# deepseek-ai/DeepEP

Measured on AMD Instinct MI355X. Metric: combine GB/s (device-resident BF16 top-k weighted reduce) at 1/2/4/8 MI355X, higher is better.
Workload: dtype bf16; 1 GPU; EP=1 combine, 8192 tokens/rank x hidden 7168 x top-8, 256 experts, uniform routing, expanded layout, gating-weighted; hidden=7168, topk=8, experts=256, accumulate=fp32, parallelism=ep1

## Files before the change

deepep_amd/_lib.py:

```python
import ctypes
import hashlib
import os
import threading
from typing import Optional

_HERE = os.path.dirname(os.path.abspath(__file__))
LIB_PATH = os.environ.get('DEEPEP_AMD_LIB', os.path.join(_HERE, 'libdeepep_amd.so'))
SOURCES = [os.path.join(_HERE, 'csrc', f) for f in ('combine.hip', 'dispatch.hip', 'symmetric.hip', 'plan.hip',
                                                      'fp8_cast.hip', 'fault.h')]
HEADER = os.path.join(os.path.dirname(_HERE), 'include', 'deepep_amd.h')
HIPCC_FLAGS = ['--offload-arch=gfx950', '-O3', '-fPIC', '-std=c++17', '-Wall']


def source_build_id() -> Optional[str]:
    if not all(os.path.exists(p) for p in SOURCES + [HEADER]):
        return None
    h = hashlib.sha256(' '.join(HIPCC_FLAGS).encode())
    for p in SOURCES + [HEADER]:
        h.update(os.path.basename(p).encode())
        with open(p, 'rb') as f:
            h.update(f.read())
    return h.hexdigest()[:16]


def binary_build_id(path: str) -> Optional[str]:
    if not os.path.exists(path):
        return None
    with open(path, 'rb') as f:
        data = f.read()
    i = data.find(b'DEEPEP_BUILD_ID=')
    return data[i + 16:i + 32].decode(errors='replace') if i >= 0 else None
ABI_VERSION = 14

MODE_LOCAL, MODE_EPILOGUE, MODE_FUSED = 0, 1, 2

ERROR_RECORD_INTS = 8
FLAG_BAD_SLOT, FLAG_TIMEOUT, FLAG_BAD_ADDRESS = 1, 2, 4
FAULT_NAMES = {1: 'scatter row outside every window', 2: 'plan window row past its window',
               3: 'plan unit / received row out of range', 4: 'dispatch row past its destination buffer'}


def describe_error_record(rec) -> str:
    rec = [int(v) for v in rec]
    bits = [n for b, n in ((FLAG_BAD_SLOT, 'rejected slot / unit'), (FLAG_TIMEOUT, 'barrier timeout'),
                           (FLAG_BAD_ADDRESS, 'address outside every window')) if rec[0] & b]
    text = f'error flag {rec[0]} ({", ".join(bits) or "none"})'
    if len(rec) > 6 and rec[1]:
        addr = (rec[5] & 0xffffffff) << 32 | (rec[4] & 0xffffffff)
        text += (f'; first fault: {FAULT_NAMES.get(rec[1], rec[1])}, unit/row {rec[2]}, rank/lane {rec[3]}, '
                 f'address {addr:#x}, extent {rec[6]}')
    return text

PLAN_BLOCK_TOKENS = 64
DISPATCH_BLOCK_ROWS = 128
PLAN_EXPANDED, PLAN_SINGLE, PLAN_INTERLEAVE, PLAN_RANK_LAYOUT, PLAN_WINDOW, PLAN_LOCAL_BYPASS = 1, 2, 4, 8, 16, 32

_lib = None
_lock = threading.Lock()

_P = ctypes.c_void_p
_I = ctypes.c_int
_I64 = ctypes.c_int64

SIGNATURES = {
    'deepep_amd_abi_version': (_I, []),
    'deepep_amd_last_error': (ctypes.c_char_p, []),
    'deepep_amd_build_id': (ctypes.c_char_p, []),
    'deepep_combine_reduce': (_I, [_I, _I,
                                   _P, _I64, _I64,
                                   _P, _I64, _I,
                                   _P,
                                   _P, _P,
                                   _P, _I64,
                                   _I, _I,
                                   _P, _I64,
                                   _P, _P, _I,
                                   _I64, _I,
                                   _I, _P,
                                   _P]),
    'deepep_build_local_plan': (_I, [_P, _I, _I, _I, _I, _P, _I, _I, _P, _P, _P]),
    'deepep_set_launch_config': (_I, [_I, _I]),
    'deepep_combine_buffer_size': (_I64, [_I, _I, _I, _I, _I]),
    'deepep_dispatch_route': (_I, [_P, _I, _I, _I, _I, _P, _P, _P, _P]),
    'deepep_dispatch_notify': (_I, [_P, _I, _I, _I, _I, _I, _P, _P, _P, _P, _I64, _P]),
    'deepep_dispatch_notify_workspace': (_I64, [_I, _I, _I]),
    'deepep_dispatch_receive': (_I, [_P, _I64, _I, _I, _I, _I, _I, _I, _P, _I, _I, _P, _I, _I, _P, _P, _P, _P, _I, _I, _P,
                                     _P, _P, _P]),
    'deepep_dispatch_expert_counts': (_I, [_P, _I, _I, _I, _P, _P]),
    'deepep_dispatch_pack': (_I, [_P, _I64, _I, _P, _I64, _I, _P, _P, _I, _I, _I, _P, _P, _I,
                                  _P, _P, _I64, _I64, _I, _I, _I, _I, _P, _P]),
    'deepep_cast_fp8': (_I, [_P, _I64, _I, _I, _I, _P, _P, _P]),
    'deepep_dispatch_pack_cast': (_I, [_P, _I64, _I, _I, _P, _P, _I, _I, _I, _P, _P, _I,
                                       _P, _P, _I64, _I64, _I, _I, _I, _I, _P, _P]),
    'deepep_dispatch_count': (_I, [_P, _I64, _I, _I, _I, _I, _I, _I, _P, _I, _I, _P, _I, _I, _P, _P, _P, _P, _P]),
    'deepep_dispatch_scan': (_I, [_P, _I, _I, _I, _I, _P, _P, _P]),
    'deepep_dispatch_slots': (_I, [_P, _I64, _I, _I, _I, _I, _I, _P, _P, _P, _P, _P]),
    'deepep_dispatch_copy': (_I, [_P, _I64, _I, _I, _I, _I, _I, _I, _P, _I, _P, _I64, _P, _I64, _I,
                                  _P, _P, _P, _I64, _P, _P, _P, _I, _P, _P, _P]),
    'deepep_route_block_counts': (_I, [_P, _I, _I, _I, _I, _I, _P, _P, _P]),
    'deepep_plan_expert': (_I, [_P, _I, _I, _I, _I, _I, _P, _P, _I, _I, _I, _P, _P, _P, _I64, _I64, _P, _P, _I,
                                _P]),
    'deepep_plan_source': (_I, [_P, _I, _I, _I, _I, _I, _I, _P, _P, _P, _I, _I, _I, _I64, _I64, _P, _I, _P, _I, _P]),
    'deepep_sym_alloc': (_I, [_I64, ctypes.POINTER(ctypes.c_void_p)]),
    'deepep_sym_free': (_I, [_P]),
    'deepep_sym_export': (_I, [_P, _P]),
    'deepep_sym_import': (_I, [_P, ctypes.POINTER(ctypes.c_void_p)]),
    'deepep_sym_close': (_I, [_P]),
    'deepep_sym_barrier': (_I, [_P, _I, _I, _I64, _I64, _P, _P]),
    'deepep_sym_put': (_I, [_P, _I64, _P, _I, _I64, _I64, _P, _P]),
    'deepep_sym_signal': (_I, [_P, _I, _I, _I, _I64, _P]),
    'deepep_sym_wait': (_I, [_P, _I, _I, _I, _I64, _I64, _P, _P]),
    'deepep_stream_create_cu_budget': (_I, [_I, ctypes.POINTER(ctypes.c_void_p)]),
    'deepep_stream_destroy': (_I, [_P]),
    'deepep_stream_probe_cus': (_I, [_P, ctypes.POINTER(ctypes.c_int), ctypes.POINTER(ctypes.c_int)]),
    'deepep_combine_reduce_scatter': (_I, [_I, _P, _I64, _I64, _P, _I64, _I, _P, _P, _I, _I, _P, _I64, _P, _I,
                                           _I64, _I, _P, _I, _I64, _P, _P]),
}


class LibraryMissing(RuntimeError):
    pass


def load(path: Optional[str] = None):
    global _lib
    with _lock:
        if _lib is not None and path is None:
            return _lib
        p = path or LIB_PATH
        if not os.path.exists(p):
            raise LibraryMissing(f'deepep_amd: HIP library not found at {p}; run __graft_entry__.build()')
        want = source_build_id() if path is None and 'DEEPEP_AMD_LIB' not in os.environ else None
        if want is not None and binary_build_id(p) != want:
            raise RuntimeError(f'deepep_amd: {p} was built from other sources (build id {binary_build_id(p)}, '
                               f'sources {want}); run __graft_entry__.build()')
        lib = ctypes.CDLL(p)
        for name, (res, args) in SIGNATURES.items():
            fn = getattr(lib, name)
            fn.restype = res
            fn.argtypes = args
        version = lib.deepep_amd_abi_version()
        if version != ABI_VERSION:
            raise RuntimeError(f'deepep_amd: ABI version {version} != expected {ABI_VERSION}')
        if path is None:
            _lib = lib
        return lib


def check(rc: int, what: str) -> None:
    if rc != 0:
        msg = load().deepep_amd_last_error().decode(errors='replace')
        raise RuntimeError(f'deepep_amd: {what} failed ({rc}): {msg}')


def ptr(t) -> Optional[int]:
    return None if t is None else t.data_ptr()
```

deepep_amd/buffer.py:

```python
import math
import os
from typing import List, Optional, Sequence, Tuple, Union

import torch
import torch.distributed as dist

from .event import EventHandle, EventOverlap
from .exchange import ExchangeMixin
from .handle import BlockCounts, CombinePlan, EPHandle, build_ep_plan, chunk_geometry
from ._lib import DISPATCH_BLOCK_ROWS
from .kernels import MODE_EPILOGUE, MODE_FUSED, MODE_LOCAL, RowLayout
from .utils import align, ceil_div, check_torch_deterministic, value_or

topk_idx_t = torch.int32 if int(os.environ.get('EP_NUM_TOPK_IDX_BITS', 64)) == 32 else torch.int64

BUFFER_ALIGNMENT = 2 * 1024 * 1024
_BUDGET_STREAMS = {}
_TOKEN_ALIGN = 32


def _assert(cond: bool, msg: str = '') -> None:
    if not cond:
        raise RuntimeError(f'Assertion failed: {msg}')


def _token_bytes(hidden_bytes: int, sf_bytes: int, num_topk: int, with_metadata: bool) -> int:
    meta = num_topk * 8 + ((1 + num_topk) * 4 if with_metadata else 0)
    return (align(hidden_bytes, _TOKEN_ALIGN) + align(sf_bytes, _TOKEN_ALIGN) + align(meta, _TOKEN_ALIGN))


def calculate_buffer_size(num_ranks: int, num_max_tokens_per_rank: int, hidden: int, num_topk: int,
                          use_fp8_dispatch: bool, allow_multiple_reduction: bool) -> int:
    _assert(num_max_tokens_per_rank > 0 and hidden > 0, 'num_max_tokens_per_rank > 0 and hidden > 0')
    num_topk = 32 if num_topk == 0 else num_topk
    elem = 1 if use_fp8_dispatch else 2
    num_sf_packs = ceil_div(hidden, 32) if use_fp8_dispatch else 0
    dispatch_bytes = num_ranks * num_max_tokens_per_rank * _token_bytes(hidden * elem, num_sf_packs * 4, num_topk, True)
    slots = min(num_ranks, num_topk) if allow_multiple_reduction else num_topk
    combine_bytes = slots * num_max_tokens_per_rank * _token_bytes(hidden * 2, 0, num_topk, False)
    return align(max(dispatch_bytes, combine_bytes), BUFFER_ALIGNMENT)


def notify_layout(notify: List[int], num_ranks: int, rank: int, experts_per_rank: int, all_gathered: bool,
                  num_blocks: int = 0):
    R, r, w = num_ranks, rank, 1 + experts_per_rank + 2 * num_blocks
    if all_gathered:
        grid = [[notify[(s * R + d) * w:(s * R + d + 1) * w] for d in range(R)] for s in range(R)]
        rows = [grid[s][r] for s in range(R)]
        sends = [grid[r][d][0] for d in range(R)]
        offsets = [sum(grid[s][d][0] for s in range(r)) for d in range(R)]
    else:
        rows = [notify[i * w:(i + 1) * w] for i in range(R)]
        sends, offsets = None, None
    recv = [row[0] for row in rows]
    experts = [sum(row[1 + e] for row in rows) for e in range(experts_per_rank)]
    blocks = [list(row[1 + experts_per_rank:]) for row in rows]
    return sends, recv, experts, offsets, blocks


class ElasticBuffer(ExchangeMixin):

    def __init__(self,
                 group: dist.ProcessGroup,
                 num_bytes: Optional[int] = None,
                 num_cpu_bytes: int = 0,
                 num_max_tokens_per_rank: int = 0,
                 hidden: int = 0,
                 num_topk: int = 0,
                 use_fp8_dispatch: bool = False,
                 deterministic: bool = False,
                 allow_hybrid_mode: bool = True,
                 allow_multiple_reduction: bool = True,
                 prefer_overlap_with_compute: bool = True,
                 sl_idx: int = 3,
                 num_allocated_qps: int = 0,
                 num_cpu_timeout_secs: int = 300, num_gpu_timeout_secs: int = 100,
                 explicitly_destroy: bool = False):
        self.group = group
        self.rank_idx = group.rank()
        self.num_ranks = group.size()
        self.allow_hybrid_mode = allow_hybrid_mode
        self.allow_multiple_reduction = allow_multiple_reduction
        self.prefer_overlap_with_compute = prefer_overlap_with_compute
        self.deterministic = deterministic
        _assert(num_cpu_bytes == 0, 'CPU buffer segments (Engram storage) are not supported by this build')
        if num_bytes is None:
            num_bytes = calculate_buffer_size(self.num_ranks, num_max_tokens_per_rank, hidden, num_topk,
                                              use_fp8_dispatch, allow_multiple_reduction)
        _assert(num_bytes % BUFFER_ALIGNMENT == 0, 'num_bytes must be aligned to 2 MB')
        if os.environ.get('EP_BUFFER_DEBUG', 0):
            print(f'Initializing EP elastic buffer with {num_bytes} bytes at rank EP {self.rank_idx}/{self.num_ranks}')
        self.num_bytes = num_bytes
        self.num_max_tokens_per_rank = num_max_tokens_per_rank
        if num_allocated_qps == 0:
            num_allocated_qps = 17 if not allow_hybrid_mode else 65
        self.num_allocated_qps = num_allocated_qps
        self.num_cpu_timeout_secs = num_cpu_timeout_secs
        self.num_gpu_timeout_secs = num_gpu_timeout_secs
        self.explicitly_destroy = explicitly_destroy
        self.num_scaleout_ranks, self.num_scaleup_ranks = 1, self.num_ranks
        self.scaleout_rank_idx, self.scaleup_rank_idx = 0, self.rank_idx
        self.num_rdma_ranks, self.num_nvlink_ranks = 1, self.num_ranks
        self.use_cuda = torch.cuda.is_available()
        self.device = torch.device('cuda', torch.cuda.current_device()) if self.use_cuda else torch.device('cpu')
        self.comm_stream = torch.cuda.Stream(device=self.device) if self.use_cuda else None
        self._kernels = None
        self.runtime = self
        self._phase_events = None
        self._phase_unpipelined = False
        self.transport = os.environ.get('DEEPEP_TRANSPORT', 'rccl')
        _assert(self.transport in ('rccl', 'xgmi'), 'DEEPEP_TRANSPORT must be rccl or xgmi')
        self.local_bypass = os.environ.get('DEEPEP_LOCAL_BYPASS', '1') != '0'
        self.phase_a_cus = int(os.environ.get('DEEPEP_PHASE_A_CUS', 0))
        self.combine_cu_mode = os.environ.get('DEEPEP_COMBINE_CUS', 'chip')
        _assert(self.combine_cu_mode in ('chip', 'handle'), 'DEEPEP_COMBINE_CUS must be chip or handle')
        self._sym = None
        self._sym_gen = None
        self._old_sym_gens = set()
        self._capturing = False
        self._sym_exchange = None
        self._group_barrier()
        if self.transport == 'xgmi' and self.num_ranks > 1 and self.use_cuda and \
                int(os.environ.get('DEEPEP_EAGER_WINDOW', 1)) and not hasattr(group, 'comm'):
            self._window(self._window_bytes(hidden, num_topk, num_max_tokens_per_rank), slots=1, rows_per_slot=1)

    class _HostCopy:

        def __init__(self, src: torch.Tensor, pinned: torch.Tensor, stream):
            self.buf = pinned[:src.numel()]
            self.buf.copy_(src, non_blocking=True)
            self.event = torch.cuda.Event()
            self.event.record(stream)

        def wait(self) -> List[int]:
            self.event.synchronize()
            return self.buf.tolist()

    def _host_copy(self, src: torch.Tensor, stream) -> '_HostCopy':
        n = src.numel()
        prev = getattr(self, '_host_copy_last', None)
        if prev is not None:
            prev.event.synchronize()
        if getattr(self, '_pinned', None) is None or self._pinned.numel() < n:
            self._pinned = torch.empty((max(n, 4096),), dtype=torch.int32, pin_memory=True)
        self._host_copy_last = ElasticBuffer._HostCopy(src, self._pinned, stream)
        return self._host_copy_last

    def _group_barrier(self) -> None:
        if self.use_cuda:
            torch.cuda.synchronize()
        if isinstance(self.group, dist.ProcessGroup):
            dist.barrier(group=self.group)
        else:
            self.group.barrier()
        if self.use_cuda:
            torch.cuda.synchronize()

    def _window_bytes(self, hidden: int, num_topk: int, num_max_tokens: int) -> int:
        if hidden <= 0 or num_max_tokens <= 0:
            return 0
        from .handle import packed_row_layout
        K = num_topk or 32
        R = self.num_ranks
        slots, single = (min(R, K), False) if self.allow_multiple_reduction else (K, True)
        combine = slots * num_max_tokens * packed_row_layout(hidden, K, True, single)[0]
        dispatch = R * num_max_tokens * max(RowLayout.make(hidden * 2, 0, K).row_bytes,
                                            RowLayout.make(hidden, ceil_div(hidden, 128) * 4, K).row_bytes)
        return max(combine, dispatch)

    @property
    def kernels(self):
        if self._kernels is None:
            from .kernels import HipKernels
            self._kernels = HipKernels()
        return self._kernels

    def destroy(self) -> None:
        assert self.explicitly_destroy
        if self.runtime is not None:
            if self.use_cuda:
                torch.cuda.synchronize()
            if self._sym is not None:
                self._group_barrier()
                self._sym.destroy()
                self._sym = None
            self.runtime = None

    @staticmethod
    def get_buffer_size_hint(group: dist.ProcessGroup, num_max_tokens_per_rank: int, hidden: int,
                             num_topk: int = 0, use_fp8_dispatch: bool = False,
                             allow_hybrid_mode: bool = True, allow_multiple_reduction: bool = True) -> int:
        return calculate_buffer_size(group.size(), num_max_tokens_per_rank, hidden, num_topk,
                                     use_fp8_dispatch, allow_multiple_reduction)

    @staticmethod
    def get_elastic_buffer_alignment() -> int:
        return BUFFER_ALIGNMENT

    def barrier(self, use_comm_stream: bool = True, with_cpu_sync: bool = False, sequential: bool = True) -> None:
        self._note_capture()
        if with_cpu_sync and self.use_cuda:
            torch.cuda.synchronize()
        rccl = isinstance(self.group, dist.ProcessGroup) and dist.get_backend(self.group) == 'nccl'
        if self.use_cuda and (self._sym is not None or rccl):
            compute = torch.cuda.current_stream()
            stream = self.comm_stream if use_comm_stream else compute
            if stream != compute:
                stream.wait_stream(compute)
            if self._sym is not None:
                if not self._capturing:
                    self._sym.poll()
                self._sym.barrier(stream)
                if not self._capturing:
                    self._sym.publish(stream)
            else:
                with torch.cuda.stream(stream):
                    dist.all_reduce(torch.zeros(1, dtype=torch.int32, device=self.device), group=self.group)
            if stream != compute:
                compute.wait_stream(stream)
        elif isinstance(self.group, dist.ProcessGroup):
            dist.barrier(group=self.group)
        else:
            self.group.barrier()
        if with_cpu_sync and self.use_cuda:
            torch.cuda.synchronize()

    @staticmethod
    def capture() -> EventHandle:
        return EventHandle()

    def get_comm_stream(self) -> torch.cuda.Stream:
        return self.comm_stream

    def get_physical_domain_size(self) -> Tuple[int, int]:
        return self.num_rdma_ranks, self.num_nvlink_ranks

    def get_logical_domain_size(self) -> Tuple[int, int]:
        return self.num_scaleout_ranks, self.num_scaleup_ranks

    def get_theoretical_num_sms(self, num_experts: int, num_topk: int, num_scaleout_topk: int = 0,
                                rdma_gbs: float = 0, nvlink_gbs: float = 0,
                                sm_read_gbs: float = 200, sm_write_gbs: float = 50) -> int:
        assert num_scaleout_topk == 0
        key = (num_experts, num_topk, rdma_gbs, nvlink_gbs, sm_read_gbs, sm_write_gbs, self.prefer_overlap_with_compute,
               os.environ.get('EP_XGMI_GBS'))
        memo = self.__dict__.setdefault('_num_sms_memo', {})
        if key in memo:
            return memo[key]
        nvlink_gbs = nvlink_gbs or float(os.environ.get('EP_XGMI_GBS', 7 * 64))
        num_device_sms = torch.cuda.get_device_properties(self.device).multi_processor_count if self.use_cuda else 256

        def expected_topk(groups: int) -> float:
            return groups * (1 - math.comb(num_experts - num_experts // groups, num_topk) / math.comb(num_experts, num_topk))

        num_sms = num_device_sms
        if self.num_ranks > 1:
            e_topk = expected_topk(self.num_ranks)
            sm_read = 1 / e_topk
            sm_write = self.num_nvlink_ranks / self.num_ranks
            traffic = self.num_nvlink_ranks / self.num_ranks * (1 - 1 / self.num_nvlink_ranks)
            num_sms = max(nvlink_gbs / traffic * sm_read / sm_read_gbs, nvlink_gbs / traffic * sm_write / sm_write_gbs)
        num_sms = align(max(4, math.ceil(num_sms * 1.25)), 2)
        num_sms = num_sms if self.prefer_overlap_with_compute else max(num_sms, 64)
        memo[key] = min(num_sms, num_device_sms)
        return memo[key]

    def get_theoretical_num_qps(self, num_sms: int) -> int:
        num_qps = min(num_sms, 8 + 1)
        if self.allow_hybrid_mode:
            num_qps = num_sms * 16 + 1
        return min(num_qps, self.num_allocated_qps)

    def _sync_mode(self, previous_event, previous_event_before_epilogue, async_with_compute_stream,
                   allocate_on_comm_stream) -> bool:
        return (not async_with_compute_stream and previous_event is None and
                previous_event_before_epilogue is None and not allocate_on_comm_stream)

    def _note_capture(self) -> None:
        self._capturing = self.use_cuda and torch.cuda.is_current_stream_capturing()

    def _prologue(self, previous_event: Optional[EventHandle], allocate_on_comm_stream: bool):
        if not self.use_cuda:
            return None
        compute_stream = torch.cuda.current_stream()
        if allocate_on_comm_stream:
            torch.cuda.set_stream(self.comm_stream)
        if previous_event is not None:
            _assert(allocate_on_comm_stream, 'previous_event requires allocate_on_comm_stream')
            previous_event.stream_wait(self.comm_stream)
        else:
            self.comm_stream.wait_stream(compute_stream)
        return compute_stream

    def _before_epilogue(self, previous_event_before_epilogue: Optional[EventHandle]) -> None:
        if previous_event_before_epilogue is not None and self.use_cuda:
            previous_event_before_epilogue.stream_wait(self.comm_stream)

    def _epilogue(self, tensors: Sequence[Optional[torch.Tensor]], compute_stream,
                  allocate_on_comm_stream: bool, async_with_compute_stream: bool) -> Optional[EventHandle]:
        if not self.use_cuda:
            return None
        event = None
        if async_with_compute_stream:
            event = EventHandle(self.comm_stream)
            if int(os.environ.get('EP_AVOID_RECORD_STREAM', 0)):
                event.tensors_to_record = list(tensors)
            else:
                for t in tensors:
                    if t is not None and t.is_cuda:
                        t.record_stream(compute_stream)
                        t.record_stream(self.comm_stream)
        else:
            compute_stream.wait_stream(self.comm_stream)
        if allocate_on_comm_stream:
            torch.cuda.set_stream(compute_stream)
        return event

    def _mark(self, stream) -> None:
        if self._phase_events is not None and self.use_cuda:
            ev = torch.cuda.Event(enable_timing=True)
            ev.record(stream)
            self._phase_events.append(ev)

    @staticmethod
    def _null_ctx():
        import contextlib
        return contextlib.nullcontext()

    def _stream_ctx(self):
        if self.use_cuda:
            return torch.cuda.stream(self.comm_stream)
        import contextlib
        return contextlib.nullcontext()

    def _a2a(self, out: torch.Tensor, inp: torch.Tensor, out_splits: Optional[List[int]] = None,
             in_splits: Optional[List[int]] = None) -> None:
        if self.num_ranks == 1:
            out.copy_(inp)
            return
        dist.all_to_all_single(out, inp, out_splits, in_splits, group=self.group)

    def _all_to_all(self, out: torch.Tensor, inp: torch.Tensor, out_splits: List[int], in_splits: List[int]) -> None:
        o = out.view(torch.uint8).view(out.shape[0], out.shape[1] * out.element_size())
        i = inp.view(torch.uint8).view(inp.shape[0], inp.shape[1] * inp.element_size())
        self._a2a(o, i, out_splits, in_splits)

    def dispatch(self,
                 x: Union[torch.Tensor, Tuple[torch.Tensor, torch.Tensor]],
                 topk_idx: Optional[torch.Tensor] = None,
                 topk_weights: Optional[torch.Tensor] = None,
                 cumulative_local_expert_recv_stats: Optional[torch.Tensor] = None,
                 num_experts: Optional[int] = None,
                 num_max_tokens_per_rank: Optional[int] = None,
                 expert_alignment: Optional[int] = None,
                 num_sms: int = 0, num_qps: int = 0,
                 previous_event: Optional[EventHandle] = None,
                 previous_event_before_epilogue: Optional[EventHandle] = None,
                 async_with_compute_stream: bool = False,
                 allocate_on_comm_stream: bool = False,
                 handle: Optional[EPHandle] = None,
                 do_handle_copy: bool = True,
                 do_cpu_sync: Optional[bool] = None,
                 do_expand: bool = False,
                 do_zero_padding: bool = False,
                 use_tma_aligned_col_major_sf: bool = False):
        check_torch_deterministic()
        args = (x, topk_idx, topk_weights, cumulative_local_expert_recv_stats, num_experts, num_max_tokens_per_rank,
                expert_alignment, num_sms, num_qps, previous_event, previous_event_before_epilogue,
                async_with_compute_stream, allocate_on_comm_stream, handle, do_handle_copy, do_cpu_sync, do_expand,
                do_zero_padding, use_tma_aligned_col_major_sf)
        budget = self._cu_budget_stream(num_sms)
        if budget is not None and self.use_cuda and torch.cuda.current_stream() == budget:
            budget = None
        if budget is None:
            return self._dispatch(*args)
        capturing = torch.cuda.is_current_stream_capturing()
        saved, self.comm_stream = self.comm_stream, budget
        if not capturing:
            budget.wait_stream(saved)
        try:
            return self._dispatch(*args, force_comm_stream=True)
        finally:
            self.comm_stream = saved
            if not capturing:
                saved.wait_stream(budget)

    def _dispatch(self, x, topk_idx, topk_weights, cumulative_local_expert_recv_stats, num_experts,
                  num_max_tokens_per_rank, expert_alignment, num_sms, num_qps, previous_event,
                  previous_event_before_epilogue, async_with_compute_stream, allocate_on_comm_stream, handle,
                  do_handle_copy, do_cpu_sync, do_expand, do_zero_padding, use_tma_aligned_col_major_sf,
                  force_comm_stream: bool = False):
        num_topk = (handle.topk_idx if topk_idx is None else topk_idx).shape[1]
        num_sms = self.get_theoretical_num_sms(num_experts or handle.num_experts, num_topk) if num_sms == 0 else num_sms
        num_qps = self.get_theoretical_num_qps(num_sms) if num_qps == 0 else num_qps
        _assert(num_qps <= self.num_allocated_qps, 'Allocated QPs are not enough')
        x, sf = x if isinstance(x, tuple) else (x, None)
        if handle is not None:
            _assert(topk_idx is None, 'topk_idx must be None with a cached handle')
            _assert(do_cpu_sync is None or not do_cpu_sync, 'Cannot do CPU sync with cached handle')
            topk_idx = handle.topk_idx
            num_max_tokens_per_rank = value_or(num_max_tokens_per_rank, handle.num_max_tokens_per_rank)
            num_experts = value_or(num_experts, handle.num_experts)
            expert_alignment = value_or(expert_alignment, handle.expert_alignment)
            do_cpu_sync = False
            _assert((num_experts, expert_alignment, num_max_tokens_per_rank) ==
                    (handle.num_experts, handle.expert_alignment, handle.num_max_tokens_per_rank),
                    'cached handle context mismatch')
            do_expand = handle.do_expand if do_expand is None else do_expand
        num_max_tokens_per_rank = value_or(num_max_tokens_per_rank, self.num_max_tokens_per_rank)
        expert_alignment = value_or(expert_alignment, 1)
        do_cpu_sync = value_or(do_cpu_sync, True)

        T, H = x.shape
        R, r = self.num_ranks, self.rank_idx
        _assert(num_experts is not None and num_experts % R == 0, 'num_experts must be divisible by the rank count')
        _assert(topk_idx.dim() == 2 and topk_idx.shape[0] == T and topk_idx.dtype == topk_idx_t,
                'topk_idx must be [num_tokens, num_topk] of deep_ep.topk_idx_t')
        _assert(T <= num_max_tokens_per_rank, 'num_tokens exceeds num_max_tokens_per_rank')
        _assert(not do_zero_padding or do_expand, 'do_zero_padding requires do_expand')
        if topk_weights is not None:
            _assert(topk_weights.shape == topk_idx.shape and topk_weights.dtype == torch.float32,
                    'topk_weights must be float32 [num_tokens, num_topk]')
        K = num_topk
        epr = num_experts // R
        self._note_capture()
        sync_mode = self._sync_mode(previous_event, previous_event_before_epilogue, async_with_compute_stream,
                                    allocate_on_comm_stream) and not force_comm_stream
        compute_stream = None if sync_mode else self._prologue(previous_event, allocate_on_comm_stream)
        kern = self.kernels
        with (self._null_ctx() if sync_mode else self._stream_ctx()):
            dev = x.device
            stream = torch.cuda.current_stream() if self.use_cuda else None
            if sync_mode and self.use_cuda and R > 1 and self.transport == 'xgmi' and not self._capturing:
                for other in [self.comm_stream, getattr(self, '_stream_b', None)] + \
                        [v[1] for k, v in _BUDGET_STREAMS.items() if k[0] == self.device.index]:
                    if other is not None and other != stream:
                        stream.wait_stream(other)
            idx64 = topk_idx if topk_idx.dtype == torch.int64 else topk_idx.to(torch.int64)
            idx64 = idx64.contiguous()
            w = topk_weights.contiguous() if topk_weights is not None else None
            cached = handle if handle is not None and (handle._send_counts is not None or
                                                       getattr(handle, '_sync_free', False)) else None
            if handle is not None:
                _assert(do_expand == handle.do_expand, 'do_expand must match the cached handle')
            worst_handle = cached is not None and getattr(cached, '_sync_free', False)
            sync_free = cached is None and not do_cpu_sync
            use_xgmi = R > 1 and self.transport == 'xgmi' and self.use_cuda
            peer_offsets = None
            host_notify = None
            counts = cached._counts if cached is not None else None
            x_bytes = x.contiguous().view(torch.uint8).view(T, H * x.element_size())
            sf_bytes = sf.contiguous().view(torch.uint8).view(T, sf.shape[1] * sf.element_size()) if sf is not None else None
            direct = R == 1
            layout = (RowLayout.make(0, 0, K) if direct else
                      RowLayout.make(x_bytes.shape[1], sf_bytes.shape[1] if sf is not None else 0, K))
            sym = self._window(layout.row_bytes, slots=R, rows_per_slot=num_max_tokens_per_rank) if use_xgmi else None
            if cached is not None:
                dst_slot = cached.dst_buffer_slot_idx
                send_counts_l, recv_counts_l = cached._send_counts, cached._recv_counts
                send_offsets = cached._send_offsets
                peer_offsets = getattr(cached, '_peer_offsets', None)
                if use_xgmi and peer_offsets is not None:
                    sym.barrier(stream)
                use_xgmi = use_xgmi and peer_offsets is not None
                _assert(not (worst_handle and R > 1) or use_xgmi == (peer_offsets is not None) and
                        (use_xgmi or cached._row_map is not None),
                        'a handle from dispatch(do_cpu_sync=False) is cached only on the transport that made it')
            else:
                nb = chunk_geometry(num_max_tokens_per_rank, 1)[0] if R > 1 else 0
                w_n = 1 + epr + 2 * nb
                dst_slot = torch.empty((T, R), dtype=torch.int32, device=dev)
                send_offsets = torch.empty((R,), dtype=torch.int32, device=dev)
                notify = torch.empty((R, w_n), dtype=torch.int32, device=dev)
                kern.dispatch_notify(idx64, num_experts, R, nb, dst_slot, notify, send_offsets, stream=stream)
                if R == 1:
                    recv_notify = notify
                elif use_xgmi:
                    rec_w = align(R + w_n, 4)
                    rec = torch.zeros((R, rec_w), dtype=torch.int32, device=dev)
                    rec[:, :R] = notify[:, 0].view(1, R)
                    rec[:, R:R + w_n] = notify
                    sym.barrier(stream)
                    sym.put_notify(rec, stream)
                    sym.barrier(stream)
                    area = sym.notify_area(rec_w)
                    recv_notify = area[:, R:R + w_n].clone()
                    peer_offsets = (area[:r, :R].sum(dim=0, dtype=torch.int32) if r > 0 else
                                    torch.zeros((R,), dtype=torch.int32, device=dev))
                else:
                    recv_notify = torch.empty_like(notify)
                    self._a2a(recv_notify, notify)
                if sync_free:
                    send_counts_l, recv_counts_l = ([T], [num_max_tokens_per_rank]) if R == 1 else (None, None)
                    expert_counts_l = own_tok = own_pairs = recv_blk = None
                elif R == 1 and self.use_cuda:
                    host_notify = self._host_copy(notify.view(-1), stream)
                    send_counts_l = recv_counts_l = [T]
                else:
                    flat = notify.view(-1) if R == 1 else torch.cat([notify.view(-1), recv_notify.reshape(-1)])
                    host = [int(v) for v in flat.tolist()]
                    own, rec_host = host[:R * w_n], (host if R == 1 else host[R * w_n:])
                    send_counts_l = own[0::w_n]
                    own_tok = [own[d * w_n + 1 + epr:d * w_n + 1 + epr + nb] for d in range(R)]
                    own_pairs = [own[d * w_n + 1 + epr + nb:(d + 1) * w_n] for d in range(R)]
                    _, recv_counts_l, expert_counts_l, _, recv_blk = notify_layout(
                        rec_host, R, r, epr, all_gathered=False, num_blocks=nb)
                counts = None
                if R > 1:
                    own_b = notify[:, 1 + epr:].reshape(R, 2, nb).transpose(0, 1)
                    rb = recv_notify[:, 1 + epr:].reshape(R, 2, nb).transpose(0, 1)
                    dev_counts = torch.cat([own_b, rb]).contiguous()
                    if sync_free:
                        counts = BlockCounts(nb, None, None, None, None, dev_counts)
                    else:
                        counts = BlockCounts(nb, own_tok, own_pairs, [b[:nb] for b in recv_blk],
                                             [b[nb:] for b in recv_blk], dev_counts)
                recv_counts_t = recv_notify[:, 0]
            N = num_max_tokens_per_rank * R if sync_free or worst_handle else sum(recv_counts_l)
            padded = (sync_free or worst_handle) and R > 1 and not use_xgmi
            pad_rows = num_max_tokens_per_rank if padded else 0
            row_map = None
            own_first = False
            if use_xgmi:
                kern.dispatch_pack(x_bytes, sf_bytes, idx64, w, r * num_max_tokens_per_rank, dst_slot,
                                   peer_offsets, None, layout, dest_bases=sym.data_bases_dev,
                                   dest_rows=sym.data_bytes // layout.row_bytes, error_flag=sym.error_flag,
                                   stream=stream)
                sym.barrier(stream)
                if not self._capturing:
                    sym.publish(stream)
                recv_packed = sym.data[:N * layout.row_bytes].view(N, layout.row_bytes)
            elif padded:
                T_max = num_max_tokens_per_rank
                own_first = cached._bypass if cached is not None else self.local_bypass
                ar = torch.arange(R, dtype=torch.int32, device=dev)
                if own_first:
                    pad_offsets = torch.where(ar == r, R - 1, torch.where(ar > r, ar - 1, ar)) * T_max
                    rows_all = torch.empty(((2 * R - 1) * T_max, layout.row_bytes), dtype=torch.uint8, device=dev)
                    kern.dispatch_pack(x_bytes, sf_bytes, idx64, w, r * T_max, dst_slot, pad_offsets, rows_all, layout,
                                       stream=stream)
                    splits = [0 if d == r else T_max for d in range(R)]
                    self._a2a(rows_all[R * T_max:], rows_all[:(R - 1) * T_max], splits, splits)
                    recv_packed = rows_all[(R - 1) * T_max:]
                else:
                    packed = torch.empty((R * T_max, layout.row_bytes), dtype=torch.uint8, device=dev)
                    kern.dispatch_pack(x_bytes, sf_bytes, idx64, w, r * T_max, dst_slot, ar * T_max, packed, layout,
                                       stream=stream)
                    recv_packed = torch.empty_like(packed)
                    self._a2a(recv_packed, packed)
                row_map = torch.empty((N,), dtype=torch.int32, device=dev)
            elif R > 1 and (cached._bypass if cached is not None else self.local_bypass):
                own = send_counts_l[r]
                n_send = sum(send_counts_l)
                if cached is None:
                    off, acc = [0] * R, 0
                    for d in [d for d in range(R) if d != r] + [r]:
                        off[d], acc = acc, acc + send_counts_l[d]
                    send_offsets = torch.tensor(off, dtype=torch.int32, device=dev)
                    row_map = torch.empty((N,), dtype=torch.int32, device=dev)
                rows_all = torch.empty((n_send + N - own, layout.row_bytes), dtype=torch.uint8, device=dev)
                kern.dispatch_pack(x_bytes, sf_bytes, idx64, w, r * num_max_tokens_per_rank, dst_slot, send_offsets,
                                   rows_all, layout, stream=stream)
                self._a2a(rows_all[n_send:], rows_all[:n_send - own],
                          [0 if d == r else c for d, c in enumerate(recv_counts_l)],
                          [0 if d == r else c for d, c in enumerate(send_counts_l)])
                recv_packed = rows_all[n_send - own:]
                own_first = True
            else:
                n_send = T if sync_free else sum(send_counts_l)
                packed = torch.empty((n_send, layout.row_bytes), dtype=torch.uint8, device=dev)
                kern.dispatch_pack(x_bytes[:, :0] if direct else x_bytes, None if direct else sf_bytes, idx64, w,
                                   r * num_max_tokens_per_rank, dst_slot, send_offsets, packed, layout, stream=stream)
                if R == 1:
                    recv_packed = packed
                else:
                    recv_packed = torch.empty((N, layout.row_bytes), dtype=torch.uint8, device=dev)
                    self._a2a(recv_packed, packed, recv_counts_l, send_counts_l)
            inv = block_offsets = None
            if cached is not None:
                psum_rank = cached.psum_num_recv_tokens_per_scaleup_rank
                psum_expert = cached.psum_num_recv_tokens_per_expert
                meta = cached.recv_src_metadata[:N]
                inv, block_offsets = getattr(cached, '_copy_tables', (None, None))
                copy_meta, copy_rows = getattr(cached, '_copy_meta', None) or (meta, N)
                row_map = getattr(cached, '_row_map', None)
                out_idx = None if do_expand else cached._recv_topk_idx[:N].clone()
                aligned_l = cached.num_recv_tokens_per_expert_list
                expert_counts = cached.num_unaligned_recv_tokens_per_expert
                if cumulative_local_expert_recv_stats is not None:
                    cumulative_local_expert_recv_stats += expert_counts.to(cumulative_local_expert_recv_stats.dtype)
                self._before_epilogue(previous_event_before_epilogue)
            else:
                psum_rank = torch.empty((R,), dtype=torch.int32, device=dev)
                meta = torch.empty((N, K + 2), dtype=torch.int32, device=dev)
                out_idx = None if do_expand else torch.empty((N, K), dtype=torch.int64, device=dev)
                nblocks = (N + DISPATCH_BLOCK_ROWS - 1) // DISPATCH_BLOCK_ROWS
                block_counts = torch.empty((nblocks, epr), dtype=torch.int32, device=dev)
                expert_counts = torch.empty((epr,), dtype=torch.int32, device=dev)
                psum_expert = torch.empty((epr,), dtype=torch.int32, device=dev)
                inv = torch.empty((N * min(K, epr) + (expert_alignment - 1) * epr,), dtype=torch.int32,
                                  device=dev) if do_expand else None
                block_offsets = block_counts if do_expand else None
                kern.dispatch_receive(recv_packed, layout, N, r, epr, recv_counts_t, psum_rank, meta, out_idx,
                                      block_counts, expert_alignment, do_expand, expert_counts, psum_expert, inv=inv,
                                      pad_rows=pad_rows, row_map=row_map, own_first=own_first, stream=stream)
                aligned_l = [] if sync_free or host_notify is not None else \
                    [align(c, expert_alignment) for c in expert_counts_l]
                if cumulative_local_expert_recv_stats is not None:
                    cumulative_local_expert_recv_stats += expert_counts.to(cumulative_local_expert_recv_stats.dtype)
                self._before_epilogue(previous_event_before_epilogue)
                copy_meta, copy_rows = meta, N
            num_unaligned = expert_counts
            deferred = host_notify is not None
            worst_tokens = num_max_tokens_per_rank * R if sync_free else T
            if do_expand and cached is not None:
                num_expanded = cached.num_expanded_tokens
                alloc = torch.zeros if do_zero_padding else torch.empty
                n_rows = num_expanded
            elif do_expand and (sync_free or deferred):
                num_expanded = align(worst_tokens * min(K, epr) + (expert_alignment - 1) * epr, expert_alignment)
                alloc = torch.zeros if do_zero_padding else torch.empty
                n_rows = num_expanded
            elif do_expand:
                num_expanded = sum(aligned_l)
                alloc = torch.zeros if do_zero_padding else torch.empty
                n_rows = num_expanded
            else:
                num_expanded = N
                alloc = torch.zeros if sync_free or worst_handle else torch.empty
                n_rows = N
            out_x = alloc((n_rows, H), dtype=x.dtype, device=dev)
            out_sf = alloc((n_rows, sf.shape[1]), dtype=sf.dtype, device=dev) if sf is not None else None
            out_w = None
            if topk_weights is not None:
                exact = expert_alignment == 1 and (bool(cached.num_recv_tokens_per_expert_list)
                                                   if cached is not None else not sync_free)
                out_w = ((torch.empty if exact else torch.zeros)((n_rows,), dtype=torch.float32, device=dev)
                         if do_expand else alloc((N, K), dtype=torch.float32, device=dev))
            kern.dispatch_copy(recv_packed, layout, copy_rows if do_expand else N, copy_meta if do_expand else meta,
                               do_expand,
                               out_x.view(torch.uint8), out_sf.view(torch.uint8) if out_sf is not None else None,
                               out_w, x_direct=x_bytes if direct else None,
                               sf_direct=sf_bytes if direct else None, num_max_tokens=num_max_tokens_per_rank,
                               error_flag=sym.error_flag if use_xgmi else None,
                               inv=inv if do_expand else None, block_offsets=block_offsets if do_expand else None,
                               expert_end=psum_expert if do_expand else None, row_map=row_map, stream=stream)
            if deferred:
                host = host_notify.wait()
                send_counts_l = recv_counts_l = [host[0]]
                expert_counts_l = host[1:1 + epr]
                aligned_l = [align(c, expert_alignment) for c in expert_counts_l]
                N = host[0]
                n_rows = sum(aligned_l) if do_expand else N
                num_expanded = n_rows if do_expand else N
                meta = meta[:N]
                out_idx = out_idx[:N] if out_idx is not None else None
                out_x = out_x[:n_rows]
                out_sf = out_sf[:n_rows] if out_sf is not None else None
                out_w = out_w[:n_rows] if out_w is not None else None
            if out_sf is not None and use_tma_aligned_col_major_sf:
                n_sf, packs = out_sf.shape
                col_major = torch.empty_strided((n_sf, packs), (1, align(max(n_sf, 1), max(1, 16 // out_sf.element_size()))),
                                                dtype=out_sf.dtype, device=dev)
                col_major.copy_(out_sf)
                out_sf = col_major
            recv_idx64 = out_idx
            if out_idx is not None and topk_idx.dtype != torch.int64:
                out_idx = out_idx.to(topk_idx.dtype)
            num_recv = N
            cloned_idx = topk_idx.clone() if do_handle_copy and cached is None else topk_idx
        event = None if sync_mode else self._epilogue([x, sf, topk_idx, topk_weights, out_x, out_sf, out_idx, out_w,
                                                       meta], compute_stream, allocate_on_comm_stream,
                                                      async_with_compute_stream)
        is_cached = handle is not None
        if not is_cached:
            handle = EPHandle(do_expand, num_experts, expert_alignment, num_max_tokens_per_rank, num_sms,
                              cloned_idx, num_recv, num_expanded, aligned_l, psum_rank, psum_expert,
                              num_unaligned, meta, dst_slot, None, None)
            handle._recv_counts = recv_counts_l
            handle._send_counts = send_counts_l
            handle._send_offsets = send_offsets
            handle._peer_offsets = peer_offsets
            handle._recv_topk_idx = recv_idx64
            handle._counts = counts
            handle._copy_tables = (inv, block_offsets)
            handle._copy_meta = (copy_meta, copy_rows) if copy_rows != N else None
            handle._row_map = row_map
            handle._bypass = own_first
            handle._sync_free = sync_free
        out_x = (out_x, out_sf) if out_sf is not None else out_x
        return out_x, out_idx, out_w, handle, EventOverlap(event)

    @staticmethod
    def _unpack_bias(bias) -> Tuple[Optional[torch.Tensor], Optional[torch.Tensor]]:
        bias_0, bias_1 = None, None
        if isinstance(bias, torch.Tensor):
            bias_0 = bias
        elif isinstance(bias, tuple):
            assert len(bias) == 2
            bias_0, bias_1 = bias
        return bias_0, bias_1

    def _num_chunks(self, handle: EPHandle) -> int:
        if self.num_ranks == 1 or (self._phase_events is not None and self._phase_unpipelined):
            return 1
        env = os.environ.get('DEEPEP_COMBINE_CHUNKS')
        if env:
            return max(1, int(env))
        return 4 if self.use_cuda and handle.num_max_tokens_per_rank >= 1024 else 1

    def _plan(self, handle: EPHandle, single_reduction: bool, num_chunks: int, hidden: int,
              window=None) -> CombinePlan:
        R = self.num_ranks
        if R == 1:
            key = ('single' if single_reduction else 'multi', 1)
        elif window is None:
            key = ('single' if single_reduction else 'multi', R, num_chunks, hidden, self.local_bypass)
        else:
            for k in [k for k in handle._combine_plans if k[0] == 'xgmi' and k[-1] in self._old_sym_gens]:
                del handle._combine_plans[k]
            key = ('xgmi', single_reduction, R, num_chunks, hidden, self._sym_gen)
        plan = handle._combine_plans.get(key)
        stream = torch.cuda.current_stream() if self.use_cuda else None
        if plan is not None:
            plan.poll()
            if self.use_cuda and not self._capturing and plan.ready is not None and plan.ready[0] != stream:
                stream.wait_event(plan.ready[1])
            return plan
        T, K = handle.topk_idx.shape
        if R == 1:
            meta = handle.recv_src_metadata
            n_recv = handle.num_recv_tokens if handle._recv_counts is None else sum(handle._recv_counts)
            plan = CombinePlan(num_ranks=1, num_tokens=T, num_topk=K, expanded=handle.do_expand)
            width = K if handle.do_expand else 1
            plan.local_table = torch.empty((T, width), dtype=torch.int32, device=meta.device)
            if not handle.do_expand:
                plan.local_wtable = torch.empty((T, K), dtype=torch.int32, device=meta.device)
            self.kernels.build_local_plan(meta, n_recv, K, handle.num_max_tokens_per_rank, handle.do_expand,
                                          plan.local_table, T, handle.topk_idx, plan.local_wtable, stream=stream)
        else:
            _assert(handle._counts is not None, 'the EP > 1 combine needs a handle made by this build\'s dispatch')
            plan = build_ep_plan(self.kernels, handle, num_ranks=R, rank=self.rank_idx, single=single_reduction,
                                 num_chunks=num_chunks, hidden=hidden, window=window, stream=stream,
                                 local_bypass=self.local_bypass)
        if not self._capturing:
            if self.use_cuda:
                ev = torch.cuda.Event()
                ev.record(stream)
                plan.ready = (stream, ev)
                plan.publish(stream)
            handle._combine_plans[key] = plan
        return plan

    def combine(self,
                x: torch.Tensor,
                handle: EPHandle,
                topk_weights: Optional[torch.Tensor] = None,
                bias: Union[torch.Tensor, Tuple[torch.Tensor, torch.Tensor]] = None,
                num_sms: int = 0, num_qps: int = 0,
                previous_event: Optional[EventHandle] = None,
                previous_event_before_epilogue: Optional[EventHandle] = None,
                async_with_compute_stream: bool = False,
                allocate_on_comm_stream: bool = False,
                *,
                apply_topk_weights: bool = False) \
            -> Tuple[torch.Tensor, Optional[torch.Tensor], EventOverlap]:
        check_torch_deterministic()
        explicit_sms = num_sms
        if num_sms == 0 and self.combine_cu_mode == 'handle' and self.prefer_overlap_with_compute:
            explicit_sms = handle.num_sms
        num_sms = handle.num_sms if num_sms == 0 else num_sms
        num_qps = self.get_theoretical_num_qps(num_sms) if num_qps == 0 else num_qps
        _assert(num_qps <= self.num_allocated_qps, 'Allocated QPs are not enough')
        bias_0, bias_1 = self._unpack_bias(bias)
        budget = self._cu_budget_stream(explicit_sms)
        if budget is not None and self.use_cuda and torch.cuda.current_stream() == budget:
            budget = None
        if budget is None:
            return self._combine(x, topk_weights, bias_0, bias_1, handle, num_sms, previous_event,
                                 previous_event_before_epilogue, async_with_compute_stream,
                                 allocate_on_comm_stream, apply_topk_weights)
        capturing = torch.cuda.is_current_stream_capturing()
        saved, self.comm_stream = self.comm_stream, budget
        if not capturing:
            budget.wait_stream(saved)
        try:
            return self._combine(x, topk_weights, bias_0, bias_1, handle, num_sms, previous_event,
                                 previous_event_before_epilogue, async_with_compute_stream,
                                 allocate_on_comm_stream, apply_topk_weights, force_comm_stream=True)
        finally:
            self.comm_stream = saved
            if not capturing:
                saved.wait_stream(budget)

    def get_cu_budget_stream(self, num_sms: int) -> Optional[torch.cuda.Stream]:
        return self._cu_budget_stream(num_sms)

    def _cu_budget_stream(self, num_sms: int):
        if num_sms <= 0 or not self.use_cuda:
            return None
        if num_sms >= torch.cuda.get_device_properties(self.device).multi_processor_count:
            return None
        key = (self.device.index, (num_sms + 7) // 8 * 8)
        if key not in _BUDGET_STREAMS:
            import ctypes
            from . import _lib
            raw = ctypes.c_void_p()
            _lib.check(self.kernels.lib.deepep_stream_create_cu_budget(key[1], ctypes.byref(raw)), 'cu_budget stream')
            _BUDGET_STREAMS[key] = (raw.value, torch.cuda.ExternalStream(raw.value, device=self.device))
        return _BUDGET_STREAMS[key][1]

    def _combine(self, x, topk_weights, bias_0, bias_1, handle, num_sms, previous_event,
                 previous_event_before_epilogue, async_with_compute_stream, allocate_on_comm_stream,
                 apply_topk_weights, force_comm_stream=False):
        _assert(self.runtime is not None, 'buffer destroyed')
        _assert(num_sms > 0, 'num_sms > 0')
        _assert(x.dim() == 2 and x.is_contiguous() and x.dtype == torch.bfloat16, 'x must be contiguous bf16 [N, hidden]')
        num_tokens, hidden = x.shape
        _assert((hidden * x.element_size()) % 16 == 0, 'hidden * sizeof(bf16) must be a multiple of 16')
        topk_idx = handle.topk_idx
        _assert(topk_idx.dim() == 2 and topk_idx.is_contiguous() and topk_idx.dtype == topk_idx_t, 'topk_idx layout')
        T, K = topk_idx.shape
        psum = handle.psum_num_recv_tokens_per_scaleup_rank
        _assert(psum.dim() == 1 and psum.shape[0] == self.num_scaleup_ranks and psum.dtype == torch.int32,
                'psum_num_recv_tokens_per_scaleup_rank must be int32 [num_scaleup_ranks]')
        _assert(T <= handle.num_max_tokens_per_rank, 'num_combined_tokens <= num_max_tokens_per_rank')
        meta = handle.recv_src_metadata
        _assert(meta.dim() == 2 and meta.shape[1] == K + 2 and meta.dtype == torch.int32 and meta.is_contiguous(),
                'recv_src_metadata must be contiguous int32 [num_recv_tokens, num_topk + 2]')
        expanded = handle.do_expand
        if not expanded:
            _assert(meta.shape[0] == num_tokens, 'non-expanded x must have one row per received token')
        if topk_weights is not None:
            if expanded:
                _assert(topk_weights.dim() == 1 and topk_weights.shape[0] == num_tokens, 'expanded weights are [N]')
            else:
                _assert(topk_weights.dim() == 2 and tuple(topk_weights.shape) == (num_tokens, K), 'weights are [N, K]')
            _assert(topk_weights.is_contiguous() and topk_weights.dtype == torch.float32, 'weights must be float32')
        for b in (bias_0, bias_1):
            if b is not None:
                _assert(b.dim() == 2 and b.is_contiguous() and b.dtype == x.dtype and tuple(b.shape) == (T, hidden),
                        'bias must be contiguous bf16 [num_combined_tokens, hidden]')
        single_reduction = expanded and not self.allow_multiple_reduction
        if single_reduction:
            _assert(topk_weights is None or apply_topk_weights,
                    'expanded combine without multiple reduction cannot carry top-k weights')
        if apply_topk_weights:
            _assert(expanded and topk_weights is not None,
                    'apply_topk_weights needs the expanded layout and topk_weights')

        kern = self.kernels
        R = self.num_ranks
        self._note_capture()
        sync_mode = self._sync_mode(previous_event, previous_event_before_epilogue, async_with_compute_stream,
                                    allocate_on_comm_stream) and not force_comm_stream
        if sync_mode:
            compute_stream = None
            stream = torch.cuda.current_stream() if self.use_cuda else None
        else:
            compute_stream = self._prologue(previous_event, allocate_on_comm_stream)
            stream = self.comm_stream
        with (self._null_ctx() if sync_mode else self._stream_ctx()):
            use_xgmi = R > 1 and self.transport == 'xgmi' and self.use_cuda
            if use_xgmi and sync_mode and not self._capturing:
                for other in [self.comm_stream, getattr(self, '_stream_b', None)] + \
                        [v[1] for k, v in _BUDGET_STREAMS.items() if k[0] == self.device.index]:
                    if other is not None and other != stream:
                        stream.wait_stream(other)
            num_chunks = self._num_chunks(handle)
            plan = None if use_xgmi else self._plan(handle, single_reduction, num_chunks, hidden)
            combined_x = torch.empty((T, hidden), dtype=x.dtype, device=x.device)
            combined_w = torch.empty((T, K), dtype=torch.float32, device=x.device) if topk_weights is not None else None
            row_w = topk_weights if apply_topk_weights else None
            wsrc = topk_weights.view(-1) if topk_weights is not None else None
            if R == 1:
                self._before_epilogue(previous_event_before_epilogue)
                if single_reduction:
                    kern.combine_reduce(MODE_EPILOGUE, x, combined_x, T, table=plan.local_table, row_weights=row_w,
                                        bias0=bias_0, bias1=bias_1, wtable=plan.local_table, wsrc=wsrc,
                                        out_weights=combined_w, stream=stream)
                else:
                    wtable = plan.local_table if expanded else plan.local_wtable
                    kern.combine_reduce(MODE_FUSED, x, combined_x, T, table=plan.local_table, row_weights=row_w,
                                        bias0=bias_0, bias1=bias_1, wtable=wtable, wsrc=wsrc,
                                        out_weights=combined_w, stream=stream)
            elif single_reduction and use_xgmi:
                self._combine_xgmi_single(handle, x, row_w, wsrc, K, hidden, bias_0, bias_1, topk_weights,
                                          combined_x, combined_w, previous_event_before_epilogue, stream)
            elif single_reduction:
                self._combine_single_chunks(plan, x, row_w, wsrc, hidden, bias_0, bias_1, combined_x, combined_w,
                                            previous_event_before_epilogue, stream)
            elif use_xgmi:
                self._combine_xgmi(handle, x, expanded, row_w, wsrc, K, hidden, bias_0, bias_1, topk_weights,
                                   combined_x, combined_w, previous_event_before_epilogue, stream)
            else:
                self._combine_chunks(plan, x, expanded, row_w, wsrc, K, hidden, bias_0, bias_1, topk_weights,
                                     combined_x, combined_w, previous_event_before_epilogue, stream)
        event = None
        if not sync_mode:
            event = self._epilogue([x, topk_weights, bias_0, bias_1, meta, topk_idx, combined_x, combined_w, psum],
                                   compute_stream, allocate_on_comm_stream, async_with_compute_stream)
        return combined_x, combined_w, EventOverlap(event)
```

deepep_amd/csrc/dispatch.hip:

```cpp
#include <hip/hip_runtime.h>
#include <stdint.h>

#include <stdio.h>

#include <algorithm>

#include "../../include/deepep_amd.h"
#include "fault.h"

extern "C" __attribute__((visibility("hidden"))) int deepep_amd_set_error(int code, const char* msg);

namespace {

typedef uint32_t u32x4 __attribute__((ext_vector_type(4)));

constexpr int kBlockRows = DEEPEP_DISPATCH_BLOCK_ROWS;

__device__ __forceinline__ uint64_t route_mask(const int64_t* __restrict__ topk_idx, int t, int T, int K, int epr) {
    uint64_t mask = 0;
    if (t < T)
        for (int k = 0; k < K; ++k) {
            const int64_t e = topk_idx[static_cast<int64_t>(t) * K + k];
            if (e >= 0) mask |= 1ull << static_cast<int>(e / epr);
        }
    return mask;
}

__global__ void __launch_bounds__(256)
route_count_kernel(const int64_t* __restrict__ topk_idx, int T, int K, int epr, int R,
                   int32_t* __restrict__ block_counts) {
    __shared__ int32_t s_cnt[4][64];
    const int tid = threadIdx.x, wave = tid >> 6, lane = tid & 63;
    const uint64_t mask = route_mask(topk_idx, blockIdx.x * 256 + tid, T, K, epr);
    for (int r = 0; r < R; ++r) {
        const int c = __popcll(__ballot((mask >> r) & 1ull));
        if (lane == 0) s_cnt[wave][r] = c;
    }
    __syncthreads();
    if (tid < R)
        block_counts[static_cast<int64_t>(blockIdx.x) * R + tid] = s_cnt[0][tid] + s_cnt[1][tid] + s_cnt[2][tid] +
                                                                   s_cnt[3][tid];
}

__global__ void __launch_bounds__(256)
route_assign_kernel(const int64_t* __restrict__ topk_idx, int T, int K, int epr, int R,
                    const int32_t* __restrict__ block_counts, int32_t* __restrict__ dst_slot,
                    int32_t* __restrict__ send_counts) {
    __shared__ int32_t s_base[64];
    __shared__ int32_t s_cnt[4][64];
    const int tid = threadIdx.x, wave = tid >> 6, lane = tid & 63;
    const int b = blockIdx.x, nb = gridDim.x;
    if (tid < R) {
        int base = 0;
        for (int j = 0; j < b; ++j) base += block_counts[static_cast<int64_t>(j) * R + tid];
        s_base[tid] = base;
        if (b == nb - 1) send_counts[tid] = base + block_counts[static_cast<int64_t>(b) * R + tid];
    }
    const int t = b * 256 + tid;
    const uint64_t mask = route_mask(topk_idx, t, T, K, epr);
    for (int r = 0; r < R; ++r) {
        const int c = __popcll(__ballot((mask >> r) & 1ull));
        if (lane == 0) s_cnt[wave][r] = c;
    }
    __syncthreads();
    if (t >= T) return;
    const uint64_t lt = lane == 0 ? 0ull : (~0ull >> (64 - lane));
    for (int r = 0; r < R; ++r) {
        const bool hit = (mask >> r) & 1ull;
        const uint64_t bal = __ballot(hit);
        int slot = -1;
        if (hit) {
            slot = s_base[r] + __popcll(bal & lt);
            for (int w = 0; w < wave; ++w) slot += s_cnt[w][r];
        }
        dst_slot[static_cast<int64_t>(t) * R + r] = slot;
    }
}

constexpr int kHistEntries = 2048;

__global__ void __launch_bounds__(256)
expert_hist_kernel(const int64_t* __restrict__ topk_idx, int64_t n, int E, int32_t* __restrict__ counts) {
    extern __shared__ int32_t s_hist[];
    for (int e = threadIdx.x; e < E; e += 256) s_hist[e] = 0;
    __syncthreads();
    const int64_t base = static_cast<int64_t>(blockIdx.x) * kHistEntries;
    for (int j = threadIdx.x; j < kHistEntries; j += 256) {
        const int64_t i = base + j;
        if (i < n) {
            const int64_t e = topk_idx[i];
            if (e >= 0 && e < E) atomicAdd(&s_hist[e], 1);
        }
    }
    __syncthreads();
    for (int e = threadIdx.x; e < E; e += 256)
        if (s_hist[e] != 0) atomicAdd(&counts[e], s_hist[e]);
}

constexpr int kNotifyTok = 256;

__global__ void __launch_bounds__(kNotifyTok)
notify_count_kernel(const int64_t* __restrict__ topk_idx, int T, int K, int E, int R, int nb,
                    int32_t* __restrict__ notify, int32_t* __restrict__ ws_cnt, int32_t* __restrict__ ws_hist) {
    extern __shared__ int32_t s_hist[];
    __shared__ int32_t s_cnt[4][64];
    const int tid = threadIdx.x, wave = tid >> 6, lane = tid & 63;
    const int epr = E / R;
    const int64_t W = 1 + epr + 2 * static_cast<int64_t>(nb);
    for (int e = tid; e < E; e += kNotifyTok) s_hist[e] = 0;
    __syncthreads();
    const int t = blockIdx.x * kNotifyTok + tid;
    uint64_t mask = 0;
    int rk[32];
#pragma unroll
    for (int k = 0; k < 32; ++k) {
        rk[k] = -1;
        if (k < K && t < T) {
            const int64_t e = topk_idx[static_cast<int64_t>(t) * K + k];
            if (e >= 0 && e < E) {
                rk[k] = static_cast<int>(e) / epr;
                mask |= 1ull << rk[k];
                atomicAdd(&s_hist[static_cast<int>(e)], 1);
            }
        }
    }
    const int b = blockIdx.x * (kNotifyTok / 64) + wave;
    for (int r = 0; r < R; ++r) {
        const uint64_t bal = __ballot((mask >> r) & 1ull);
        if (lane == 0) s_cnt[wave][r] = __popcll(bal);
        if (nb > 0) {
            int c = 0;
#pragma unroll
            for (int k = 0; k < 32; ++k) c += rk[k] == r;
#pragma unroll
            for (int off = 32; off > 0; off >>= 1) c += __shfl_xor(c, off, 64);
            if (lane == 0 && b < nb) {
                notify[r * W + 1 + epr + b] = __popcll(bal);
                notify[r * W + 1 + epr + nb + b] = c;
            }
        }
    }
    __syncthreads();
    if (tid < R)
        ws_cnt[static_cast<int64_t>(blockIdx.x) * R + tid] = s_cnt[0][tid] + s_cnt[1][tid] + s_cnt[2][tid] + s_cnt[3][tid];
    for (int e = tid; e < E; e += kNotifyTok) ws_hist[static_cast<int64_t>(blockIdx.x) * E + e] = s_hist[e];
}

__global__ void __launch_bounds__(kNotifyTok)
notify_assign_kernel(const int64_t* __restrict__ topk_idx, int T, int K, int E, int R, int nb, int nblk,
                     const int32_t* __restrict__ ws_cnt, const int32_t* __restrict__ ws_hist,
                     int32_t* __restrict__ dst_slot, int32_t* __restrict__ notify, int32_t* __restrict__ send_offsets) {
    __shared__ int32_t s_base[64];
    __shared__ int32_t s_cnt[4][64];
    const int tid = threadIdx.x, wave = tid >> 6, lane = tid & 63;
    const int blk = blockIdx.x, grid = gridDim.x;
    const int epr = E / R;
    const int64_t W = 1 + epr + 2 * static_cast<int64_t>(nb);
    constexpr int kBatch = 16;
    auto column_sum = [&](const int32_t* __restrict__ base, int64_t stride, int n) {
        int c = 0;
        for (int j0 = 0; j0 < n; j0 += kBatch) {
            int v[kBatch];
#pragma unroll
            for (int j = 0; j < kBatch; ++j) v[j] = j0 + j < n ? base[static_cast<int64_t>(j0 + j) * stride] : 0;
#pragma unroll
            for (int j = 0; j < kBatch; ++j) c += v[j];
        }
        return c;
    };
    if (tid < R) s_base[tid] = column_sum(ws_cnt + tid, R, min(blk, nblk));
    const int t = blk * kNotifyTok + tid;
    uint64_t mask = 0;
    if (t < T)
        for (int k = 0; k < K; ++k) {
            const int64_t e = topk_idx[static_cast<int64_t>(t) * K + k];
            if (e >= 0 && e < E) mask |= 1ull << (static_cast<int>(e) / epr);
        }
    for (int r = 0; r < R; ++r) {
        const int c = __popcll(__ballot((mask >> r) & 1ull));
        if (lane == 0) s_cnt[wave][r] = c;
    }
    __syncthreads();
    if (blk < nblk && t < T) {
        const uint64_t lt = lane == 0 ? 0ull : (~0ull >> (64 - lane));
        for (int r = 0; r < R; ++r) {
            const bool hit = (mask >> r) & 1ull;
            const uint64_t bal = __ballot(hit);
            int slot = -1;
            if (hit) {
                slot = s_base[r] + __popcll(bal & lt);
                for (int w = 0; w < wave; ++w) slot += s_cnt[w][r];
            }
            dst_slot[static_cast<int64_t>(t) * R + r] = slot;
        }
    }
    for (int e = blk * kNotifyTok + tid; e < E; e += grid * kNotifyTok) {
        const int r = e / epr;
        notify[r * W + 1 + (e - r * epr)] = column_sum(ws_hist + e, E, nblk);
    }
    if (blk == 0) {
        __syncthreads();
        if (tid < R) {
            const int total = column_sum(ws_cnt + tid, R, nblk);
            s_base[tid] = total;
            notify[tid * W] = total;
        }
        __syncthreads();
        if (tid < R) {
            int before = 0;
            for (int q = 0; q < tid; ++q) before += s_base[q];
            send_offsets[tid] = before;
        }
    }
    const int covered = nblk * (kNotifyTok / 64);
    for (int i = blk * kNotifyTok + tid; i < R * nb; i += grid * kNotifyTok) {
        const int r = i / nb, bb = i - r * nb;
        if (bb >= covered) {
            notify[r * W + 1 + epr + bb] = 0;
            notify[r * W + 1 + epr + nb + bb] = 0;
        }
    }
}

template <bool kPeer>
__device__ __forceinline__ void put16(uint8_t* row, int off, const u32x4& v, int row_bytes) {
    if constexpr (kPeer) {
        const __amdgpu_buffer_rsrc_t rs = __builtin_amdgcn_make_buffer_rsrc(row, 0, row_bytes, 0x00020000);
        __builtin_amdgcn_raw_buffer_store_b128(v, rs, off, 0, 17);
    } else {
        *reinterpret_cast<u32x4*>(row + off) = v;
    }
}

template <bool kPeer, typename V>
__device__ __forceinline__ void put(V* p, V v) {
    if constexpr (kPeer) __hip_atomic_store(p, v, __ATOMIC_RELAXED, __HIP_MEMORY_SCOPE_SYSTEM);
    else *p = v;
}

template <bool kPeer>
__global__ void __launch_bounds__(64)
pack_kernel(const uint8_t* __restrict__ x, int64_t x_stride, int x_bytes,
            const uint8_t* __restrict__ sf, int64_t sf_stride, int sf_bytes,
            const int64_t* __restrict__ topk_idx, const float* __restrict__ topk_weights, int K,
            int32_t src_base, const int32_t* __restrict__ dst_slot, const int32_t* __restrict__ send_offsets, int R,
            uint8_t* __restrict__ packed, const uint64_t* __restrict__ dest_bases, int64_t row_bytes,
            int64_t dest_rows, int sf_off, int idx_off, int w_off, int src_off, int32_t* __restrict__ error_flag) {
    const int t = blockIdx.x, lane = threadIdx.x;
    if (kPeer && error_flag != nullptr &&
        (__hip_atomic_load(error_flag, __ATOMIC_RELAXED, __HIP_MEMORY_SCOPE_AGENT) & 2))
        return;
    uint64_t my_row = 0;
    if (lane < R) {
        const int32_t s = dst_slot[static_cast<int64_t>(t) * R + lane];
        if (s >= 0) {
            const uint64_t base = kPeer ? dest_bases[lane] : reinterpret_cast<uint64_t>(packed);
            const int64_t row = static_cast<int64_t>(send_offsets[lane]) + s;
            if (row >= 0 && row < dest_rows)
                my_row = base + static_cast<uint64_t>(row) * row_bytes;
            else
                deepep::record_fault(error_flag, DEEPEP_FLAG_BAD_ADDRESS, DEEPEP_FAULT_PACK_ROW, t, lane,
                                     base + static_cast<uint64_t>(row) * row_bytes, dest_rows);
        }
    }
    const uint64_t dmask = __ballot(my_row != 0);
    auto row_of = [&](int r) -> uint8_t* {
        const uint64_t lo = static_cast<uint32_t>(__builtin_amdgcn_readlane(static_cast<int>(my_row & 0xffffffffu), r));
        const uint64_t hi = static_cast<uint32_t>(__builtin_amdgcn_readlane(static_cast<int>(my_row >> 32), r));
        return reinterpret_cast<uint8_t*>((hi << 32) | lo);
    };
    const u32x4* xs = reinterpret_cast<const u32x4*>(x + t * x_stride);
    for (int v = lane; v < x_bytes / 16; v += 64) {
        const u32x4 val = __builtin_nontemporal_load(xs + v);
        for (uint64_t m = dmask; m; m &= m - 1)
            put16<kPeer>(row_of(__builtin_ctzll(m)), v * 16, val, static_cast<int>(row_bytes));
    }
    for (int v = lane; v < sf_bytes / 4; v += 64) {
        const uint32_t val = reinterpret_cast<const uint32_t*>(sf + t * sf_stride)[v];
        for (uint64_t m = dmask; m; m &= m - 1)
            put<kPeer>(reinterpret_cast<uint32_t*>(row_of(__builtin_ctzll(m)) + sf_off) + v, val);
    }
    int64_t e = 0;
    float w = 0.0f;
    if (lane < K) {
        e = topk_idx[static_cast<int64_t>(t) * K + lane];
        w = topk_weights != nullptr ? topk_weights[static_cast<int64_t>(t) * K + lane] : 0.0f;
    }
    for (uint64_t m = dmask; m; m &= m - 1) {
        uint8_t* row = row_of(__builtin_ctzll(m));
        if (lane < K) {
            put<kPeer>(reinterpret_cast<int64_t*>(row + idx_off) + lane, e);
            put<kPeer>(reinterpret_cast<float*>(row + w_off) + lane, w);
        }
        if (lane == 0) put<kPeer>(reinterpret_cast<int32_t*>(row + src_off), static_cast<int32_t>(src_base + t));
    }
}

__device__ __forceinline__ int local_expert(int64_t e, int rank, int epr) {
    return (e >= static_cast<int64_t>(rank) * epr && e < static_cast<int64_t>(rank + 1) * epr)
               ? static_cast<int>(e - static_cast<int64_t>(rank) * epr) : -1;
}

__global__ void __launch_bounds__(kBlockRows)
count_kernel(const uint8_t* __restrict__ packed, int64_t row_bytes, int idx_off, int src_off, int N, int K,
             int rank, int epr, const int32_t* __restrict__ recv_counts, int counts_stride, int32_t* __restrict__ psum_out,
             int R, int pad_rows, int own_first, int32_t* __restrict__ row_map,
             int32_t* __restrict__ meta, int64_t* __restrict__ recv_topk_idx, int32_t* __restrict__ block_counts,
             int fill_slots) {
    extern __shared__ int32_t s_hist[];
    __shared__ int32_t rank_psum[64];
    for (int e = threadIdx.x; e < epr; e += kBlockRows) s_hist[e] = 0;
    if (threadIdx.x < R)
        rank_psum[threadIdx.x] = recv_counts[static_cast<int64_t>(threadIdx.x) * (counts_stride > 0 ? counts_stride : 1)];
    __syncthreads();
    if (counts_stride > 0) {
        if (threadIdx.x == 0)
            for (int s = 1; s < R; ++s) rank_psum[s] += rank_psum[s - 1];
        __syncthreads();
        if (psum_out != nullptr && blockIdx.x == 0 && threadIdx.x < R) psum_out[threadIdx.x] = rank_psum[threadIdx.x];
    }
    const int i = blockIdx.x * kBlockRows + threadIdx.x;
    const int received = min(N, rank_psum[R - 1]);
    if (i >= received && i < N) {
        const int64_t mrow = static_cast<int64_t>(i) * (K + 2);
        meta[mrow] = -1;
        meta[mrow + 1] = -1;
        if (recv_topk_idx != nullptr)
            for (int k = 0; k < K; ++k) recv_topk_idx[static_cast<int64_t>(i) * K + k] = -1;
    }
    if (i < received) {
        int src_rank = 0;
        while (src_rank < R - 1 && i >= rank_psum[src_rank]) ++src_rank;
        const int start = src_rank > 0 ? rank_psum[src_rank - 1] : 0;
        const int own_start = rank > 0 ? rank_psum[rank - 1] : 0, own_rows = rank_psum[rank] - own_start;
        int64_t prow = i;
        if (pad_rows > 0) {
            const int slot = !own_first ? src_rank : (src_rank == rank ? 0 : (src_rank < rank ? src_rank + 1 : src_rank));
            prow = static_cast<int64_t>(slot) * pad_rows + i - start;
        } else if (own_first) {
            prow = src_rank == rank ? i - own_start : (src_rank < rank ? i + own_rows : i);
        }
        if (row_map != nullptr) row_map[i] = static_cast<int32_t>(prow);
        const uint8_t* row = packed + prow * row_bytes;
        const int64_t* idx = reinterpret_cast<const int64_t*>(row + idx_off);
        int master = -1;
        for (int k = 0; k < K; ++k) {
            const int le = local_expert(idx[k], rank, epr);
            if (le >= 0) {
                master = k;
                atomicAdd(&s_hist[le], 1);
            }
            if (recv_topk_idx != nullptr) recv_topk_idx[static_cast<int64_t>(i) * K + k] = le;
        }
        const int64_t mrow = static_cast<int64_t>(i) * (K + 2);
        meta[mrow] = *reinterpret_cast<const int32_t*>(row + src_off);
        meta[mrow + 1] = src_rank * K + master;
    }
    if (fill_slots && i < N)
        for (int k = 0; k < K; ++k) meta[static_cast<int64_t>(i) * (K + 2) + 2 + k] = -1;
    __syncthreads();
    if (blockIdx.x * kBlockRows < N)
        for (int e = threadIdx.x; e < epr; e += kBlockRows)
            block_counts[static_cast<int64_t>(blockIdx.x) * epr + e] = s_hist[e];
}

__global__ void __launch_bounds__(1024)
scan_kernel(int32_t* __restrict__ block_counts, int nblocks, int epr, int align, int expanded,
            int32_t* __restrict__ expert_counts, int32_t* __restrict__ psum_expert) {
    constexpr int kBatch = 16;
    __shared__ int32_t s_part[1024];
    __shared__ int32_t s_aligned[1024];
    const int tid = threadIdx.x;
    const int G = 1024 / epr;
    const int e = tid % epr, g = tid / epr;
    const bool active = g < G;
    const int per = (nblocks + G - 1) / G;
    const int b_lo = min(nblocks, g * per), b_hi = min(nblocks, b_lo + per);
    int part = 0;
    if (active)
        for (int b0 = b_lo; b0 < b_hi; b0 += kBatch) {
            int c[kBatch];
#pragma unroll
            for (int j = 0; j < kBatch; ++j)
                c[j] = b0 + j < b_hi ? block_counts[static_cast<int64_t>(b0 + j) * epr + e] : 0;
#pragma unroll
            for (int j = 0; j < kBatch; ++j) part += c[j];
        }
    if (active) s_part[tid] = part;
    __syncthreads();
    int total = 0;
    if (tid < epr)
        for (int q = 0; q < G; ++q) total += s_part[q * epr + tid];
    const int aligned = tid < epr ? (total + align - 1) / align * align : 0;
    s_aligned[tid] = aligned;
    __syncthreads();
    for (int off = 1; off < 1024; off <<= 1) {
        const int v = tid >= off ? s_aligned[tid - off] : 0;
        __syncthreads();
        s_aligned[tid] += v;
        __syncthreads();
    }
    if (tid < epr) {
        const int start = s_aligned[tid] - aligned;
        expert_counts[tid] = total;
        psum_expert[tid] = expanded ? start + total : start + aligned;
        s_aligned[tid] = start;
    }
    __syncthreads();
    if (!active) return;
    int run = s_aligned[e];
    for (int q = 0; q < g; ++q) run += s_part[q * epr + e];
    for (int b0 = b_lo; b0 < b_hi; b0 += kBatch) {
        int c[kBatch];
#pragma unroll
        for (int j = 0; j < kBatch; ++j)
            c[j] = b0 + j < b_hi ? block_counts[static_cast<int64_t>(b0 + j) * epr + e] : 0;
#pragma unroll
        for (int j = 0; j < kBatch; ++j) {
            if (b0 + j < b_hi) block_counts[static_cast<int64_t>(b0 + j) * epr + e] = run;
            run += c[j];
        }
    }
}

constexpr int kSlotWaves = kBlockRows / 64;

__global__ void __launch_bounds__(kBlockRows)
slots_kernel(const uint8_t* __restrict__ packed, int64_t row_bytes, int idx_off, int N, int K, int rank, int epr,
             const int32_t* __restrict__ block_offsets, int32_t* __restrict__ meta, int32_t* __restrict__ inv,
             const int32_t* __restrict__ row_map) {
    extern __shared__ uint64_t s_bits[];
    for (int j = threadIdx.x; j < epr * kSlotWaves; j += kBlockRows) s_bits[j] = 0ull;
    __syncthreads();
    const int i = blockIdx.x * kBlockRows + threadIdx.x;
    const int wave = threadIdx.x >> 6, lane = threadIdx.x & 63;
    const bool valid = i < N && meta[static_cast<int64_t>(i) * (K + 2)] >= 0;
    const int64_t prow = valid && row_map != nullptr ? row_map[i] : i;
    const int64_t* idx = reinterpret_cast<const int64_t*>(packed + prow * row_bytes + idx_off);
    if (valid)
        for (int k = 0; k < K; ++k) {
            const int le = local_expert(idx[k], rank, epr);
            if (le >= 0) atomicOr(reinterpret_cast<unsigned long long*>(&s_bits[le * kSlotWaves + wave]), 1ull << lane);
        }
    __syncthreads();
    if (i >= N) return;
    const uint64_t lt = lane == 0 ? 0ull : (~0ull >> (64 - lane));
    for (int k = 0; k < K; ++k) {
        const int le = valid ? local_expert(idx[k], rank, epr) : -1;
        int slot = -1;
        if (le >= 0) {
            slot = block_offsets[static_cast<int64_t>(blockIdx.x) * epr + le];
            for (int w = 0; w < wave; ++w) slot += __popcll(s_bits[le * kSlotWaves + w]);
            slot += __popcll(s_bits[le * kSlotWaves + wave] & lt);
            if (inv != nullptr) inv[slot] = i * K + k;
        }
        meta[static_cast<int64_t>(i) * (K + 2) + 2 + k] = slot;
    }
}

__global__ void __launch_bounds__(256)
copy_kernel(const uint8_t* __restrict__ packed, int64_t row_bytes, int x_bytes, int sf_off, int sf_bytes, int w_off,
            int N, int K, const int32_t* __restrict__ meta, int expanded,
            const uint8_t* __restrict__ x_direct, int64_t x_direct_stride,
            const uint8_t* __restrict__ sf_direct, int64_t sf_direct_stride, int num_max_tokens,
            uint8_t* __restrict__ recv_x, uint8_t* __restrict__ recv_sf, float* __restrict__ recv_w,
            int64_t num_out_rows, const int32_t* __restrict__ row_map, int32_t* __restrict__ error_flag) {
    constexpr int kChunkVecs = 128;
    const int lane = threadIdx.x & 63;
    if (error_flag != nullptr && (__hip_atomic_load(error_flag, __ATOMIC_RELAXED, __HIP_MEMORY_SCOPE_AGENT) & 2))
        return;
    const int nvec = x_bytes / 16;
    const int nchunks = max(1, (nvec + kChunkVecs - 1) / kChunkVecs);
    const int64_t it = static_cast<int64_t>(blockIdx.x) * 4 + (threadIdx.x >> 6);
    if (it >= static_cast<int64_t>(N) * nchunks) return;
    const int64_t i = it / nchunks;
    const int c = static_cast<int>(it - i * nchunks);
    if (meta[i * (K + 2)] < 0) return;
    const uint8_t* row = packed + (row_map != nullptr ? static_cast<int64_t>(row_map[i]) : i) * row_bytes;
    const uint8_t* xs = row;
    const uint8_t* sfs = row + sf_off;
    if (x_direct != nullptr) {
        const int64_t t = meta[i * (K + 2)] % num_max_tokens;
        xs = x_direct + t * x_direct_stride;
        sfs = sf_direct != nullptr ? sf_direct + t * sf_direct_stride : nullptr;
    }
    int32_t my_dst = -1;
    if (expanded) {
        if (lane < K) my_dst = meta[i * (K + 2) + 2 + lane];
    } else if (lane == 0) {
        my_dst = static_cast<int32_t>(i);
    }
    if (my_dst >= num_out_rows) {
        if (error_flag != nullptr) atomicOr(error_flag, 1);
        my_dst = -1;
    }
    const uint64_t dmask = __ballot(my_dst >= 0);
    const int v0 = c * kChunkVecs + lane, v1 = v0 + 64;
    const u32x4 zero = {0u, 0u, 0u, 0u};
    const u32x4 a0 = v0 < nvec ? __builtin_nontemporal_load(reinterpret_cast<const u32x4*>(xs) + v0) : zero;
    const u32x4 a1 = v1 < nvec ? __builtin_nontemporal_load(reinterpret_cast<const u32x4*>(xs) + v1) : zero;
    for (uint64_t m = dmask; m; m &= m - 1) {
        const int64_t d = __builtin_amdgcn_readlane(my_dst, __builtin_ctzll(m));
        const __amdgpu_buffer_rsrc_t rs = __builtin_amdgcn_make_buffer_rsrc(recv_x + d * x_bytes, 0, x_bytes,
                                                                            0x00020000);
        __builtin_amdgcn_raw_buffer_store_b128(a0, rs, v0 * 16, 0, 16);
        __builtin_amdgcn_raw_buffer_store_b128(a1, rs, v1 * 16, 0, 16);
    }
    if (c != 0) return;
    if (recv_sf != nullptr && sfs != nullptr)
        for (int v = lane; v < sf_bytes / 4; v += 64) {
            const uint32_t val = reinterpret_cast<const uint32_t*>(sfs)[v];
            for (uint64_t m = dmask; m; m &= m - 1) {
                const int64_t d = __builtin_amdgcn_readlane(my_dst, __builtin_ctzll(m));
                reinterpret_cast<uint32_t*>(recv_sf + d * sf_bytes)[v] = val;
            }
        }
    if (recv_w != nullptr && lane < K) {
        const float w = reinterpret_cast<const float*>(row + w_off)[lane];
        if (expanded) {
            if (my_dst >= 0) recv_w[my_dst] = w;
        } else {
            recv_w[i * K + lane] = w;
        }
    }
}

constexpr int kCopyAux = 18;

template <bool kDirect>
__global__ void __launch_bounds__(256)
copy_expanded_kernel(const uint8_t* __restrict__ packed, int64_t row_bytes, int x_bytes, int sf_off, int sf_bytes,
                     int w_off, int N, int K, const int32_t* __restrict__ meta,
                     const uint8_t* __restrict__ x_direct, int64_t x_direct_stride,
                     const uint8_t* __restrict__ sf_direct, int64_t sf_direct_stride, int num_max_tokens,
                     const int32_t* __restrict__ inv, const int32_t* __restrict__ block_offsets,
                     const int32_t* __restrict__ expert_end, int nb, int epr,
                     uint8_t* __restrict__ recv_x, uint8_t* __restrict__ recv_sf, float* __restrict__ recv_w,
                     int64_t num_out_rows, const int32_t* __restrict__ row_map, int32_t* __restrict__ error_flag) {
    constexpr int kChunkVecs = 128;
    constexpr int kRows = 4;
    const int lane = threadIdx.x & 63, wave = threadIdx.x >> 6;
    if (error_flag != nullptr && (__hip_atomic_load(error_flag, __ATOMIC_RELAXED, __HIP_MEMORY_SCOPE_AGENT) & 2))
        return;
    const int nvec = x_bytes / 16;
    const int nch = max(1, (nvec + kChunkVecs - 1) / kChunkVecs);
    const int64_t wg_per_block = (static_cast<int64_t>(epr) * nch + 3) / 4;
    const int64_t xcd = blockIdx.x % 8, kk = blockIdx.x / 8;
    const int64_t b = xcd + 8 * (kk / wg_per_block);
    const int64_t it = (kk % wg_per_block) * 4 + wave;
    const int e = static_cast<int>(it / nch), c = static_cast<int>(it - static_cast<int64_t>(e) * nch);
    if (b >= nb || e >= epr) return;
    const int r0 = block_offsets[b * epr + e];
    const int r1 = b + 1 < nb ? block_offsets[(b + 1) * epr + e] : expert_end[e];
    const int v0 = c * kChunkVecs + lane, v1 = v0 + 64;
    const u32x4 zero = {0u, 0u, 0u, 0u};
    for (int j = r0; j < r1; j += kRows) {
        const uint8_t* rows[kRows];
        int32_t src_i[kRows], src_k[kRows];
        u32x4 a[kRows][2];
#pragma unroll
        for (int q = 0; q < kRows; ++q) {
            src_i[q] = -1;
            src_k[q] = 0;
            rows[q] = nullptr;
            if (j + q < r1) {
                const int32_t code = __builtin_amdgcn_readfirstlane(inv[j + q]);
                const int32_t i = code >= 0 ? code / K : -1;
                if (i >= 0 && i < N) {
                    src_i[q] = i;
                    src_k[q] = code - i * K;
                    if constexpr (kDirect) {
                        const int64_t t = meta[static_cast<int64_t>(i) * (K + 2)] % num_max_tokens;
                        rows[q] = x_direct + t * x_direct_stride;
                    } else {
                        rows[q] = packed + (row_map != nullptr ? static_cast<int64_t>(row_map[i]) : i) * row_bytes;
                    }
                    const u32x4* xs = reinterpret_cast<const u32x4*>(rows[q]);
                    a[q][0] = v0 < nvec ? xs[v0] : zero;
                    a[q][1] = v1 < nvec ? xs[v1] : zero;
                }
            }
        }
#pragma unroll
        for (int q = 0; q < kRows; ++q) {
            if (src_i[q] < 0) continue;
            const int64_t d = j + q;
            if (d >= num_out_rows) {
                if (lane == 0 && error_flag != nullptr) atomicOr(error_flag, 1);
                continue;
            }
            const __amdgpu_buffer_rsrc_t rs = __builtin_amdgcn_make_buffer_rsrc(recv_x + d * x_bytes, 0, x_bytes,
                                                                                0x00020000);
            __builtin_amdgcn_raw_buffer_store_b128(a[q][0], rs, v0 * 16, 0, kCopyAux);
            __builtin_amdgcn_raw_buffer_store_b128(a[q][1], rs, v1 * 16, 0, kCopyAux);
            if (c != 0) continue;
            if (recv_sf != nullptr) {
                const uint8_t* sfs;
                if constexpr (kDirect) {
                    const int64_t t = meta[static_cast<int64_t>(src_i[q]) * (K + 2)] % num_max_tokens;
                    sfs = sf_direct != nullptr ? sf_direct + t * sf_direct_stride : nullptr;
                } else {
                    sfs = rows[q] + sf_off;
                }
                if (sfs != nullptr)
                    for (int v = lane; v < sf_bytes / 4; v += 64)
                        reinterpret_cast<uint32_t*>(recv_sf + d * sf_bytes)[v] = reinterpret_cast<const uint32_t*>(sfs)[v];
            }
            if (recv_w != nullptr && lane == 0) {
                const int64_t prow = row_map != nullptr ? static_cast<int64_t>(row_map[src_i[q]]) : src_i[q];
                recv_w[d] = reinterpret_cast<const float*>(packed + prow * row_bytes + w_off)[src_k[q]];
            }
        }
    }
}

int launch_status(const char* what) {
    const hipError_t err = hipGetLastError();
    if (err != hipSuccess) {
        char buf[256];
        snprintf(buf, sizeof(buf), "%s launch failed: %s", what, hipGetErrorString(err));
        return deepep_amd_set_error(DEEPEP_ERR_HIP, buf);
    }
    return DEEPEP_OK;
}

bool a16(const void* p) { return (reinterpret_cast<uintptr_t>(p) & 15u) == 0; }

}

extern "C" {

int deepep_dispatch_route(const int64_t* topk_idx, int num_tokens, int num_topk, int num_experts, int num_ranks,
                          int32_t* dst_slot, int32_t* send_counts, int32_t* block_counts, deepep_stream_t stream) {
    if (num_tokens < 0 || num_topk < 1 || num_topk > 32 || num_ranks < 1 || num_ranks > 64 ||
        num_experts % num_ranks != 0 || send_counts == nullptr ||
        (num_tokens > 0 && (dst_slot == nullptr || topk_idx == nullptr || block_counts == nullptr)))
        return deepep_amd_set_error(DEEPEP_ERR_INVALID_ARG, "dispatch_route: invalid arguments");
    hipStream_t s = reinterpret_cast<hipStream_t>(stream);
    if (num_tokens == 0) {
        const hipError_t e = hipMemsetAsync(send_counts, 0, sizeof(int32_t) * num_ranks, s);
        return e == hipSuccess ? DEEPEP_OK : launch_status("dispatch_route memset");
    }
    const int nb = (num_tokens + 255) / 256;
    const int epr = num_experts / num_ranks;
    hipLaunchKernelGGL(route_count_kernel, dim3(nb), dim3(256), 0, s, topk_idx, num_tokens, num_topk, epr, num_ranks,
                       block_counts);
    hipLaunchKernelGGL(route_assign_kernel, dim3(nb), dim3(256), 0, s, topk_idx, num_tokens, num_topk, epr, num_ranks,
                       block_counts, dst_slot, send_counts);
    return launch_status("dispatch_route");
}

int64_t deepep_dispatch_notify_workspace(int num_tokens, int num_experts, int num_ranks) {
    const int64_t nblk = (static_cast<int64_t>(std::max(num_tokens, 0)) + kNotifyTok - 1) / kNotifyTok;
    return nblk * (num_ranks + num_experts) * 4;
}

int deepep_dispatch_notify(const int64_t* topk_idx, int num_tokens, int num_topk, int num_experts, int num_ranks,
                           int num_blocks, int32_t* dst_slot, int32_t* notify, int32_t* send_offsets,
                           void* workspace, int64_t workspace_bytes, deepep_stream_t stream) {
    if (num_tokens < 0 || num_topk < 1 || num_topk > 32 || num_ranks < 1 || num_ranks > 64 ||
        num_experts < num_ranks || num_experts % num_ranks != 0 || num_experts > 32768 ||
        num_blocks < 0 || (num_ranks > 1 && num_blocks < (num_tokens + 63) / 64) ||
        notify == nullptr || send_offsets == nullptr || (num_tokens > 0 && (dst_slot == nullptr || topk_idx == nullptr)) ||
        workspace_bytes < deepep_dispatch_notify_workspace(num_tokens, num_experts, num_ranks) ||
        (num_tokens > 0 && workspace == nullptr))
        return deepep_amd_set_error(DEEPEP_ERR_INVALID_ARG, "dispatch_notify: invalid arguments");
    hipStream_t s = reinterpret_cast<hipStream_t>(stream);
    const int nblk = (num_tokens + kNotifyTok - 1) / kNotifyTok;
    int32_t* ws_cnt = static_cast<int32_t*>(workspace);
    int32_t* ws_hist = ws_cnt + static_cast<int64_t>(nblk) * num_ranks;
    if (nblk > 0)
        hipLaunchKernelGGL(notify_count_kernel, dim3(nblk), dim3(kNotifyTok), static_cast<size_t>(num_experts) * 4, s,
                           topk_idx, num_tokens, num_topk, num_experts, num_ranks, num_blocks, notify, ws_cnt, ws_hist);
    hipLaunchKernelGGL(notify_assign_kernel, dim3(std::max(nblk, 1)), dim3(kNotifyTok), 0, s, topk_idx, num_tokens,
                       num_topk, num_experts, num_ranks, num_blocks, nblk, ws_cnt, ws_hist, dst_slot, notify,
                       send_offsets);
    return launch_status("dispatch_notify");
}

int deepep_dispatch_expert_counts(const int64_t* topk_idx, int num_tokens, int num_topk, int num_experts,
                                  int32_t* counts, deepep_stream_t stream) {
    if (num_tokens < 0 || num_topk < 1 || num_topk > 32 || num_experts < 1 || num_experts > 32768 ||
        counts == nullptr || (num_tokens > 0 && topk_idx == nullptr))
        return deepep_amd_set_error(DEEPEP_ERR_INVALID_ARG, "dispatch_expert_counts: invalid arguments");
    hipStream_t s = reinterpret_cast<hipStream_t>(stream);
    const hipError_t e = hipMemsetAsync(counts, 0, sizeof(int32_t) * num_experts, s);
    if (e != hipSuccess) return launch_status("dispatch_expert_counts memset");
    const int64_t n = static_cast<int64_t>(num_tokens) * num_topk;
    if (n > 0)
        hipLaunchKernelGGL(expert_hist_kernel, dim3(static_cast<unsigned>((n + kHistEntries - 1) / kHistEntries)),
                           dim3(256), num_experts * 4, s, topk_idx, n, num_experts, counts);
    return launch_status("dispatch_expert_counts");
}

int deepep_dispatch_pack(const void* x, int64_t x_row_stride_bytes, int x_bytes,
                         const void* sf, int64_t sf_row_stride_bytes, int sf_bytes,
                         const int64_t* topk_idx, const float* topk_weights, int num_tokens, int num_topk,
                         int32_t src_base, const int32_t* dst_slot, const int32_t* send_offsets, int num_ranks,
                         void* packed, const uint64_t* dest_bases, int64_t row_bytes, int64_t dest_rows,
                         int sf_off, int idx_off, int w_off, int src_off, int32_t* error_flag,
                         deepep_stream_t stream) {
    if (num_tokens == 0) return DEEPEP_OK;
    if (num_tokens < 0 || num_topk < 1 || num_topk > 32 || num_ranks < 1 || num_ranks > 64 || x_bytes % 16 ||
        dest_rows < 0 || row_bytes < src_off + 4 ||
        sf_bytes % 4 || row_bytes % 16 || !a16(x) || (dest_bases == nullptr && !a16(packed)) ||
        x_row_stride_bytes % 16 || idx_off % 8 || w_off % 4 || src_off % 4 || (sf_bytes > 0 && sf == nullptr) ||
        (dest_bases == nullptr && packed == nullptr))
        return deepep_amd_set_error(DEEPEP_ERR_INVALID_ARG, "dispatch_pack: invalid arguments or alignment");
    hipStream_t s = reinterpret_cast<hipStream_t>(stream);
    if (dest_bases != nullptr)
        hipLaunchKernelGGL(pack_kernel<true>, dim3(num_tokens), dim3(64), 0, s,
                           static_cast<const uint8_t*>(x), x_row_stride_bytes, x_bytes,
                           static_cast<const uint8_t*>(sf), sf_row_stride_bytes, sf_bytes,
                           topk_idx, topk_weights, num_topk, src_base, dst_slot, send_offsets, num_ranks,
                           static_cast<uint8_t*>(packed), dest_bases, row_bytes, dest_rows, sf_off, idx_off, w_off, src_off,
                           error_flag);
    else
        hipLaunchKernelGGL(pack_kernel<false>, dim3(num_tokens), dim3(64), 0, s,
                           static_cast<const uint8_t*>(x), x_row_stride_bytes, x_bytes,
                           static_cast<const uint8_t*>(sf), sf_row_stride_bytes, sf_bytes,
                           topk_idx, topk_weights, num_topk, src_base, dst_slot, send_offsets, num_ranks,
                           static_cast<uint8_t*>(packed), dest_bases, row_bytes, dest_rows, sf_off, idx_off, w_off, src_off,
                           error_flag);
    return launch_status("dispatch_pack");
}

int deepep_dispatch_count(const void* packed, int64_t row_bytes, int idx_off, int src_off, int num_recv, int num_topk,
                          int rank, int num_local_experts, const int32_t* recv_rank_psum, int num_ranks,
                          int recv_counts_stride, int32_t* psum_out, int pad_rows, int own_first, int32_t* row_map,
                          int32_t* src_metadata, int64_t* recv_topk_idx, int32_t* block_counts,
                          deepep_stream_t stream) {
    if (num_recv == 0 && (psum_out == nullptr || recv_counts_stride == 0)) return DEEPEP_OK;
    if (num_recv < 0 || num_topk < 1 || num_topk > 32 || num_local_experts < 1 || num_local_experts > 1024 ||
        num_ranks < 1 || num_ranks > 64 || recv_counts_stride < 0 || rank < 0 || rank >= num_ranks ||
        (num_recv > 0 && (src_metadata == nullptr || block_counts == nullptr || packed == nullptr)) ||
        recv_rank_psum == nullptr || pad_rows < 0 || (num_recv > 0 && (pad_rows > 0 || own_first) && row_map == nullptr) ||
        static_cast<int64_t>(pad_rows) * num_ranks >= (int64_t(1) << 31))
        return deepep_amd_set_error(DEEPEP_ERR_INVALID_ARG, "dispatch_count: invalid arguments");
    const int nblocks = std::max(1, (num_recv + kBlockRows - 1) / kBlockRows);
    hipLaunchKernelGGL(count_kernel, dim3(nblocks), dim3(kBlockRows), num_local_experts * 4,
                       reinterpret_cast<hipStream_t>(stream), static_cast<const uint8_t*>(packed), row_bytes,
                       idx_off, src_off, num_recv, num_topk, rank, num_local_experts, recv_rank_psum,
                       recv_counts_stride, psum_out, num_ranks, pad_rows, own_first ? 1 : 0, row_map, src_metadata,
                       recv_topk_idx, block_counts, 0);
    return launch_status("dispatch_count");
}

int deepep_dispatch_receive(const void* packed, int64_t row_bytes, int idx_off, int src_off, int num_recv,
                            int num_topk, int rank, int num_local_experts, const int32_t* recv_counts,
                            int num_ranks, int recv_counts_stride, int32_t* psum_out, int pad_rows, int own_first,
                            int32_t* row_map, int32_t* src_metadata, int64_t* recv_topk_idx, int32_t* block_counts,
                            int expert_alignment, int expanded, int32_t* expert_counts, int32_t* psum_expert,
                            int32_t* inv, deepep_stream_t stream) {
    if (num_recv < 0 || num_topk < 1 || num_topk > 32 || num_local_experts < 1 || num_local_experts > 1024 ||
        num_ranks < 1 || num_ranks > 64 || recv_counts_stride < 1 || recv_counts == nullptr || psum_out == nullptr ||
        rank < 0 || rank >= num_ranks ||
        (num_recv > 0 && (src_metadata == nullptr || block_counts == nullptr || packed == nullptr)) ||
        pad_rows < 0 || (num_recv > 0 && (pad_rows > 0 || own_first) && row_map == nullptr) ||
        static_cast<int64_t>(pad_rows) * num_ranks >= (int64_t(1) << 31) || expert_alignment < 1 ||
        expert_counts == nullptr || psum_expert == nullptr ||
        static_cast<int64_t>(num_recv) * num_topk >= (int64_t(1) << 31))
        return deepep_amd_set_error(DEEPEP_ERR_INVALID_ARG, "dispatch_receive: invalid arguments");
    hipStream_t s = reinterpret_cast<hipStream_t>(stream);
    const int nblocks = (num_recv + kBlockRows - 1) / kBlockRows;
    hipLaunchKernelGGL(count_kernel, dim3(std::max(nblocks, 1)), dim3(kBlockRows), num_local_experts * 4, s,
                       static_cast<const uint8_t*>(packed), row_bytes, idx_off, src_off, num_recv, num_topk, rank,
                       num_local_experts, recv_counts, recv_counts_stride, psum_out, num_ranks, pad_rows,
                       own_first ? 1 : 0, row_map, src_metadata, recv_topk_idx, block_counts, expanded ? 0 : 1);
    hipLaunchKernelGGL(scan_kernel, dim3(1), dim3(1024), 0, s, block_counts, nblocks, num_local_experts,
                       expert_alignment, expanded, expert_counts, psum_expert);
    if (expanded && nblocks > 0)
        hipLaunchKernelGGL(slots_kernel, dim3(nblocks), dim3(kBlockRows), num_local_experts * kSlotWaves * 8, s,
                           static_cast<const uint8_t*>(packed), row_bytes, idx_off, num_recv, num_topk, rank,
                           num_local_experts, block_counts, src_metadata, inv, row_map);
    return launch_status("dispatch_receive");
}

int deepep_dispatch_scan(int32_t* block_counts, int num_blocks, int num_local_experts, int expert_alignment,
                         int expanded, int32_t* expert_counts, int32_t* psum_expert, deepep_stream_t stream) {
    if (num_blocks < 0 || num_local_experts < 1 || num_local_experts > 1024 || expert_alignment < 1 ||
        expert_counts == nullptr || psum_expert == nullptr || (num_blocks > 0 && block_counts == nullptr))
        return deepep_amd_set_error(DEEPEP_ERR_INVALID_ARG, "dispatch_scan: invalid arguments");
    hipLaunchKernelGGL(scan_kernel, dim3(1), dim3(1024), 0, reinterpret_cast<hipStream_t>(stream),
                       block_counts, num_blocks, num_local_experts, expert_alignment, expanded,
                       expert_counts, psum_expert);
    return launch_status("dispatch_scan");
}

int deepep_dispatch_slots(const void* packed, int64_t row_bytes, int idx_off, int num_recv, int num_topk,
                          int rank, int num_local_experts, const int32_t* block_offsets, int32_t* src_metadata,
                          int32_t* inv, const int32_t* row_map, deepep_stream_t stream) {
    if (num_recv == 0) return DEEPEP_OK;
    if (num_recv < 0 || num_topk < 1 || num_topk > 32 || num_local_experts < 1 || num_local_experts > 1024 ||
        packed == nullptr || block_offsets == nullptr || src_metadata == nullptr ||
        static_cast<int64_t>(num_recv) * num_topk >= (int64_t(1) << 31))
        return deepep_amd_set_error(DEEPEP_ERR_INVALID_ARG, "dispatch_slots: invalid arguments");
    const int nblocks = (num_recv + kBlockRows - 1) / kBlockRows;
    hipLaunchKernelGGL(slots_kernel, dim3(nblocks), dim3(kBlockRows), num_local_experts * kSlotWaves * 8,
                       reinterpret_cast<hipStream_t>(stream), static_cast<const uint8_t*>(packed), row_bytes,
                       idx_off, num_recv, num_topk, rank, num_local_experts, block_offsets, src_metadata, inv,
                       row_map);
    return launch_status("dispatch_slots");
}

int deepep_dispatch_copy(const void* packed, int64_t row_bytes, int x_bytes, int sf_off, int sf_bytes, int w_off,
                         int num_recv, int num_topk, const int32_t* src_metadata, int expanded,
                         const void* x_direct, int64_t x_direct_stride_bytes,
                         const void* sf_direct, int64_t sf_direct_stride_bytes, int num_max_tokens,
                         void* recv_x, void* recv_sf, float* recv_topk_weights, int64_t num_out_rows,
                         const int32_t* inv, const int32_t* block_offsets, const int32_t* expert_end,
                         int num_local_experts, const int32_t* row_map, int32_t* error_flag, deepep_stream_t stream) {
    if (num_recv == 0) return DEEPEP_OK;
    if (num_recv < 0 || num_topk < 1 || num_topk > 32 || x_bytes % 16 || row_bytes % 16 || !a16(packed) ||
        num_out_rows < 0 ||
        !a16(recv_x) || (recv_sf != nullptr && sf_bytes % 4) || src_metadata == nullptr ||
        (x_direct != nullptr && (!a16(x_direct) || x_direct_stride_bytes % 16 || num_max_tokens < 1 ||
                                 (recv_sf != nullptr && sf_direct == nullptr))) ||
        (inv != nullptr && (!expanded || block_offsets == nullptr || expert_end == nullptr || num_local_experts < 1 ||
                            num_local_experts > 1024)))
        return deepep_amd_set_error(DEEPEP_ERR_INVALID_ARG, "dispatch_copy: invalid arguments or alignment");
    if (inv != nullptr) {
        const int nb = (num_recv + kBlockRows - 1) / kBlockRows;
        const int nch = std::max(1, (x_bytes / 16 + 127) / 128);
        const int64_t wg_per_block = (static_cast<int64_t>(num_local_experts) * nch + 3) / 4;
        const int64_t grid = 8 * wg_per_block * ((nb + 7) / 8);
        auto launch = [&](auto kernel) {
            hipLaunchKernelGGL(kernel, dim3(static_cast<unsigned>(grid)), dim3(256), 0,
                               reinterpret_cast<hipStream_t>(stream),
                               static_cast<const uint8_t*>(packed), row_bytes, x_bytes, sf_off, sf_bytes, w_off,
                               num_recv, num_topk, src_metadata, static_cast<const uint8_t*>(x_direct),
                               x_direct_stride_bytes, static_cast<const uint8_t*>(sf_direct), sf_direct_stride_bytes,
                               num_max_tokens, inv, block_offsets, expert_end, nb, num_local_experts,
                               static_cast<uint8_t*>(recv_x), static_cast<uint8_t*>(recv_sf), recv_topk_weights,
                               num_out_rows, row_map, error_flag);
        };
        if (x_direct != nullptr) launch(copy_expanded_kernel<true>);
        else launch(copy_expanded_kernel<false>);
        return launch_status("dispatch_copy");
    }
    const int64_t nchunks = std::max<int64_t>(1, (x_bytes / 16 + 127) / 128);
    const int64_t items = static_cast<int64_t>(num_recv) * nchunks;
    hipLaunchKernelGGL(copy_kernel, dim3(static_cast<unsigned>((items + 3) / 4)), dim3(256), 0,
                       reinterpret_cast<hipStream_t>(stream),
                       static_cast<const uint8_t*>(packed), row_bytes, x_bytes, sf_off, sf_bytes, w_off,
                       num_recv, num_topk, src_metadata, expanded,
                       static_cast<const uint8_t*>(x_direct), x_direct_stride_bytes,
                       static_cast<const uint8_t*>(sf_direct), sf_direct_stride_bytes, num_max_tokens,
                       static_cast<uint8_t*>(recv_x), static_cast<uint8_t*>(recv_sf), recv_topk_weights,
                       num_out_rows, row_map, error_flag);
    return launch_status("dispatch_copy");
}

}
```

deepep_amd/kernels.py:

```python
from dataclasses import dataclass
from typing import Optional

import torch

from . import _lib
from ._lib import MODE_EPILOGUE, MODE_FUSED, MODE_LOCAL, ptr
from .utils import align

__all__ = ['HipKernels', 'RowLayout', 'MODE_LOCAL', 'MODE_EPILOGUE', 'MODE_FUSED']


@dataclass(frozen=True)
class RowLayout:
    x_bytes: int
    sf_bytes: int
    num_topk: int
    sf_off: int
    idx_off: int
    w_off: int
    src_off: int
    row_bytes: int

    @staticmethod
    def make(x_bytes: int, sf_bytes: int, num_topk: int) -> 'RowLayout':
        sf_off = x_bytes
        idx_off = align(sf_off + sf_bytes, 16)
        w_off = idx_off + align(num_topk * 8, 16)
        src_off = w_off + align(num_topk * 4, 16)
        return RowLayout(x_bytes, sf_bytes, num_topk, sf_off, idx_off, w_off, src_off, align(src_off + 16, 128))


def _require(cond: bool, msg: str) -> None:
    if not cond:
        raise RuntimeError(f'deepep_amd: {msg}')


def _stream_handle(stream) -> int:
    return stream.cuda_stream if stream is not None else torch.cuda.current_stream().cuda_stream


def _table_view(table: Optional[torch.Tensor]):
    if table is None:
        return None, 0, 1
    _require(table.dim() == 2 and table.dtype == torch.int32 and table.stride(1) == 1,
             'slot tables must be 2-D int32 with unit column stride')
    return table, table.stride(0), table.shape[1]


class HipKernels:

    name = 'hip'

    def __init__(self):
        self.lib = _lib.load()

    def combine_reduce(self, mode: int, src: torch.Tensor, out: torch.Tensor, num_units: int,
                       table: Optional[torch.Tensor] = None,
                       row_weights: Optional[torch.Tensor] = None,
                       bias0: Optional[torch.Tensor] = None, bias1: Optional[torch.Tensor] = None,
                       wtable: Optional[torch.Tensor] = None, wsrc: Optional[torch.Tensor] = None,
                       out_weights: Optional[torch.Tensor] = None,
                       units_per_block: int = 0, error_flag: Optional[torch.Tensor] = None,
                       weights_pad: int = 0, stream=None) -> None:
        _require(src.is_cuda and out.is_cuda, 'combine tensors must be on the GPU')
        _require(src.dtype == torch.bfloat16 and out.dtype == torch.bfloat16, 'combine rows must be bfloat16')
        _require(src.dim() == 2 and out.dim() == 2 and (src.numel() == 0 or src.stride(1) == 1) and
                 (out.numel() == 0 or out.stride(1) == 1), 'combine rows must be 2-D with unit column stride')
        hidden = out.shape[1]
        _require(src.shape[1] == hidden or src.shape[0] == 0, 'source and output hidden sizes differ')
        _require(out.shape[0] >= num_units, 'output has fewer rows than units')
        for b in (bias0, bias1):
            if b is not None:
                _require(b.is_cuda and b.dtype == torch.bfloat16 and b.is_contiguous() and
                         tuple(b.shape) == (num_units, hidden), 'bias must be contiguous bf16 [num_tokens, hidden]')
        t, t_stride, t_width = _table_view(table)
        if t is not None:
            _require(t.shape[0] >= num_units, 'slot table has fewer rows than units')
        w, w_stride, _ = _table_view(wtable)
        num_weights = 0
        ow_stride = 0
        if out_weights is not None:
            _require(out_weights.dtype == torch.float32 and out_weights.dim() == 2 and out_weights.stride(1) == 1,
                     'weights must be float32 [units, k] with unit column stride')
            _require(out_weights.shape[0] >= num_units, 'weight output has fewer rows than units')
            num_weights = out_weights.shape[1]
            ow_stride = out_weights.stride(0)
            _require(wsrc is not None and wsrc.dtype == torch.float32 and wsrc.dim() == 1 and
                     (wsrc.stride(0) == 1 or wsrc.numel() <= 1), 'weight source must be a 1-D float32 view')
        weighted = row_weights is not None
        if weighted:
            _require(row_weights.dtype == torch.float32 and row_weights.is_contiguous(),
                     'row weights must be contiguous float32')
        rc = self.lib.deepep_combine_reduce(
            mode, int(weighted),
            ptr(src), src.shape[0], src.stride(0) if src.shape[0] > 0 else hidden,
            ptr(t), t_stride, t_width,
            ptr(row_weights),
            ptr(bias0), ptr(bias1),
            ptr(out), out.stride(0) if out.shape[0] > 0 else hidden,
            num_units, hidden,
            ptr(w), w_stride,
            ptr(wsrc), ptr(out_weights), num_weights, ow_stride, weights_pad,
            units_per_block, ptr(error_flag),
            _stream_handle(stream))
        _lib.check(rc, 'combine_reduce')

    def combine_reduce_scatter(self, src: torch.Tensor, num_units: int, out_rows: torch.Tensor,
                               table: Optional[torch.Tensor] = None, row_weights: Optional[torch.Tensor] = None,
                               wtable: Optional[torch.Tensor] = None, wsrc: Optional[torch.Tensor] = None,
                               num_weights: int = 0, weights_offset: int = 0, weights_pad: int = 0,
                               error_flag: Optional[torch.Tensor] = None, *, windows, stream=None) -> None:
        _require(src.is_cuda and src.dtype == torch.bfloat16 and src.dim() == 2 and
                 (src.numel() == 0 or src.stride(1) == 1), 'combine rows must be 2-D bf16 on the GPU with unit column stride')
        _require(out_rows.is_cuda and out_rows.dtype == torch.int64 and out_rows.is_contiguous() and
                 out_rows.shape[0] >= num_units, 'out_rows must be int64 [num_units] on the GPU')
        win_bases, win_bytes = windows
        _require(win_bases.is_cuda and win_bases.dtype == torch.int64 and win_bases.is_contiguous() and
                 win_bases.dim() == 1, 'window bases must be int64 [num_windows] on the GPU')
        _require(error_flag is None or error_flag.numel() >= 1, 'error flag')
        t, t_stride, t_width = _table_view(table)
        w, w_stride, _ = _table_view(wtable)
        if num_weights:
            _require(wsrc is not None and wsrc.dtype == torch.float32 and wsrc.dim() == 1, 'weight source')
        if row_weights is not None:
            _require(row_weights.dtype == torch.float32 and row_weights.is_contiguous(), 'row weights')
        hidden = src.shape[1]
        rc = self.lib.deepep_combine_reduce_scatter(
            int(row_weights is not None), ptr(src), src.shape[0], src.stride(0) if src.shape[0] > 0 else hidden,
            ptr(t), t_stride, t_width, ptr(row_weights), ptr(out_rows), num_units, hidden,
            ptr(w), w_stride, ptr(wsrc), num_weights, weights_offset, weights_pad,
            ptr(win_bases), win_bases.shape[0], int(win_bytes), ptr(error_flag), _stream_handle(stream))
        _lib.check(rc, 'combine_reduce_scatter')

    def build_local_plan(self, src_metadata: torch.Tensor, num_recv_tokens: int, num_topk: int,
                         num_max_tokens_per_rank: int, expanded: bool, plan: torch.Tensor,
                         num_tokens: int, topk_idx: Optional[torch.Tensor] = None,
                         wtable: Optional[torch.Tensor] = None, stream=None) -> None:
        _require(src_metadata.is_cuda and src_metadata.dtype == torch.int32 and src_metadata.is_contiguous(),
                 'recv_src_metadata must be contiguous int32 on the GPU')
        _require(plan.is_contiguous() and plan.dtype == torch.int32, 'plan must be contiguous int32')
        rc = self.lib.deepep_build_local_plan(
            ptr(src_metadata), num_recv_tokens, num_topk, num_max_tokens_per_rank, int(expanded),
            ptr(plan), plan.shape[1], num_tokens, ptr(topk_idx), ptr(wtable), _stream_handle(stream))
        _lib.check(rc, 'build_local_plan')

    def dispatch_route(self, topk_idx, num_experts, num_ranks, dst_slot, send_counts, stream=None):
        _require(topk_idx.is_cuda and topk_idx.dtype == torch.int64 and topk_idx.is_contiguous(), 'topk_idx int64')
        T, K = topk_idx.shape
        block_counts = torch.empty((max(1, (T + 255) // 256) * num_ranks,), dtype=torch.int32, device=topk_idx.device)
        rc = self.lib.deepep_dispatch_route(ptr(topk_idx), T, K, num_experts, num_ranks, ptr(dst_slot),
                                            ptr(send_counts), ptr(block_counts), _stream_handle(stream))
        _lib.check(rc, 'dispatch_route')

    def dispatch_notify(self, topk_idx, num_experts, num_ranks, num_blocks, dst_slot, notify, send_offsets,
                        stream=None):
        _require(topk_idx.is_cuda and topk_idx.dtype == torch.int64 and topk_idx.is_contiguous(), 'topk_idx int64')
        T, K = topk_idx.shape
        W = 1 + num_experts // num_ranks + 2 * num_blocks
        _require(notify.dtype == torch.int32 and notify.is_contiguous() and tuple(notify.shape) == (num_ranks, W),
                 'notify must be contiguous int32 [num_ranks, 1 + experts_per_rank + 2 * num_blocks]')
        _require(dst_slot.dtype == torch.int32 and dst_slot.is_contiguous() and dst_slot.numel() == T * num_ranks,
                 'dst_slot must be contiguous int32 [num_tokens, num_ranks]')
        _require(send_offsets.dtype == torch.int32 and send_offsets.is_contiguous() and
                 send_offsets.numel() == num_ranks, 'send_offsets must be contiguous int32 [num_ranks]')
        ws_bytes = int(self.lib.deepep_dispatch_notify_workspace(T, num_experts, num_ranks))
        ws = torch.empty((max(ws_bytes, 16),), dtype=torch.uint8, device=topk_idx.device)
        rc = self.lib.deepep_dispatch_notify(ptr(topk_idx), T, K, num_experts, num_ranks, num_blocks, ptr(dst_slot),
                                             ptr(notify), ptr(send_offsets), ptr(ws), ws.numel(),
                                             _stream_handle(stream))
        _lib.check(rc, 'dispatch_notify')

    def dispatch_expert_counts(self, topk_idx, num_experts, counts, stream=None):
        _require(topk_idx.is_cuda and topk_idx.dtype == torch.int64 and topk_idx.is_contiguous(), 'topk_idx int64')
        _require(counts.dtype == torch.int32 and counts.is_contiguous() and counts.numel() == num_experts,
                 'expert counts must be contiguous int32 [num_experts]')
        T, K = topk_idx.shape
        rc = self.lib.deepep_dispatch_expert_counts(ptr(topk_idx), T, K, num_experts, ptr(counts),
                                                    _stream_handle(stream))
        _lib.check(rc, 'dispatch_expert_counts')

    def route_block_counts(self, topk_idx, num_experts, num_ranks, num_blocks, tok, pairs, stream=None):
        _require(topk_idx.is_cuda and topk_idx.dtype == torch.int64 and topk_idx.is_contiguous(), 'topk_idx int64')
        for t in (tok, pairs):
            _require(t.dtype == torch.int32 and t.is_contiguous() and t.numel() == num_ranks * num_blocks,
                     'block counts must be contiguous int32 [num_ranks, num_blocks]')
        T, K = topk_idx.shape
        rc = self.lib.deepep_route_block_counts(ptr(topk_idx), T, K, num_experts, num_ranks, num_blocks, ptr(tok),
                                                ptr(pairs), _stream_handle(stream))
        _lib.check(rc, 'route_block_counts')

    def plan_expert(self, meta, num_topk, num_ranks, rank, num_max_tokens, recv_tok, recv_pairs, num_blocks,
                    blocks_per_chunk, flags, table_a, wtable_a, window_bases, window_row_bytes, out_rows,
                    window_bytes: int = 0, error_flag=None, padded_stride: int = 0, stream=None):
        _require(meta.is_cuda and meta.dtype == torch.int32 and meta.is_contiguous(), 'recv_src_metadata int32')
        _require(table_a.dtype == torch.int32 and table_a.is_contiguous(), 'table_a int32')
        _require(wtable_a is None or (wtable_a.dtype == torch.int32 and wtable_a.is_contiguous()), 'wtable_a int32')
        _require(out_rows is None or (out_rows.dtype == torch.int64 and out_rows.is_contiguous() and
                                      window_bases is not None and window_bytes > 0),
                 'out_rows int64 with window bases and extent')
        rc = self.lib.deepep_plan_expert(ptr(meta), meta.shape[0], num_topk, num_ranks, rank, num_max_tokens,
                                         ptr(recv_tok), ptr(recv_pairs), num_blocks, blocks_per_chunk, flags,
                                         ptr(table_a), ptr(wtable_a), ptr(window_bases), window_row_bytes,
                                         int(window_bytes), ptr(out_rows), ptr(error_flag), int(padded_stride),
                                         _stream_handle(stream))
        _lib.check(rc, 'plan_expert')

    def plan_source(self, topk_idx, num_experts, num_ranks, rank, num_max_tokens, dst_slot, send_tok, send_pairs,
                    num_blocks, blocks_per_chunk, flags, row_floats, weights_offset, table_b, wtable,
                    padded_stride: int = 0, stream=None):
        _require(topk_idx.is_cuda and topk_idx.dtype == torch.int64 and topk_idx.is_contiguous(), 'topk_idx int64')
        _require(table_b.dtype == torch.int32 and table_b.is_contiguous(), 'table_b int32')
        _require(wtable is None or (wtable.dtype == torch.int32 and wtable.is_contiguous()), 'wtable int32')
        T, K = topk_idx.shape
        rc = self.lib.deepep_plan_source(ptr(topk_idx), T, K, num_experts, num_ranks, rank, num_max_tokens, ptr(dst_slot),
                                         ptr(send_tok), ptr(send_pairs), num_blocks, blocks_per_chunk, flags,
                                         row_floats, weights_offset, ptr(table_b), table_b.shape[1], ptr(wtable),
                                         int(padded_stride), _stream_handle(stream))
        _lib.check(rc, 'plan_source')

    def dispatch_pack(self, x_bytes, sf_bytes, topk_idx, topk_weights, src_base, dst_slot, send_offsets,
                      packed, layout: RowLayout, dest_bases=None, dest_rows: Optional[int] = None, error_flag=None,
                      stream=None):
        T, K = topk_idx.shape
        if dest_bases is not None:
            _require(dest_bases.is_cuda and dest_bases.dtype == torch.int64 and dest_bases.is_contiguous() and
                     dest_bases.numel() == dst_slot.shape[1], 'dest_bases must be int64 [num_ranks] on the GPU')
            _require(dest_rows is not None, 'dest_rows (rows per destination window) is required with dest_bases')
        else:
            dest_rows = packed.shape[0] if dest_rows is None else min(dest_rows, packed.shape[0])
        rc = self.lib.deepep_dispatch_pack(
            ptr(x_bytes), x_bytes.stride(0) if T else layout.x_bytes, layout.x_bytes,
            ptr(sf_bytes), sf_bytes.stride(0) if sf_bytes is not None and T else 0, layout.sf_bytes,
            ptr(topk_idx), ptr(topk_weights), T, K, src_base, ptr(dst_slot), ptr(send_offsets),
            dst_slot.shape[1], ptr(packed), ptr(dest_bases), layout.row_bytes, int(dest_rows), layout.sf_off,
            layout.idx_off,
            layout.w_off, layout.src_off, ptr(error_flag), _stream_handle(stream))
        _lib.check(rc, 'dispatch_pack')

    def cast_fp8(self, x, q, sf, round_scale: bool = False, stream=None):
        _require(x.is_cuda and x.dim() == 2 and x.dtype == torch.bfloat16 and (x.numel() == 0 or x.stride(1) == 1),
                 'cast_fp8 input must be 2-D bf16 on the GPU with unit column stride')
        T, H = x.shape
        _require(H % 128 == 0, 'cast_fp8 needs a hidden size that is a multiple of 128')
        _require(q.dtype == torch.float8_e4m3fn and q.is_contiguous() and tuple(q.shape) == (T, H) and
                 sf.dtype == torch.float32 and sf.is_contiguous() and tuple(sf.shape) == (T, H // 128),
                 'cast_fp8 outputs must be contiguous float8_e4m3fn [T, H] and float32 [T, H / 128]')
        rc = self.lib.deepep_cast_fp8(ptr(x), x.stride(0) * 2 if T else H * 2, T, H, int(round_scale), ptr(q),
                                      ptr(sf), _stream_handle(stream))
        _lib.check(rc, 'cast_fp8')

    def dispatch_pack_cast(self, x_bytes, topk_idx, topk_weights, src_base, dst_slot, send_offsets, packed,
                           layout: RowLayout, round_scale: bool = False, dest_bases=None,
                           dest_rows: Optional[int] = None, error_flag=None, stream=None):
        T, K = topk_idx.shape
        H = layout.x_bytes
        _require(H % 128 == 0 and layout.sf_bytes == H // 128 * 4 and x_bytes.shape[1] == 2 * H,
                 'dispatch_pack_cast needs bf16 rows of H % 128 == 0 columns and the FP8 row layout of H')
        if dest_bases is not None:
            _require(dest_bases.is_cuda and dest_bases.dtype == torch.int64 and dest_bases.is_contiguous() and
                     dest_bases.numel() == dst_slot.shape[1], 'dest_bases must be int64 [num_ranks] on the GPU')
            _require(dest_rows is not None, 'dest_rows (rows per destination window) is required with dest_bases')
        else:
            dest_rows = packed.shape[0] if dest_rows is None else min(dest_rows, packed.shape[0])
        rc = self.lib.deepep_dispatch_pack_cast(
            ptr(x_bytes), x_bytes.stride(0) if T else 2 * H, H, int(round_scale),
            ptr(topk_idx), ptr(topk_weights), T, K, src_base, ptr(dst_slot), ptr(send_offsets),
            dst_slot.shape[1], ptr(packed), ptr(dest_bases), layout.row_bytes, int(dest_rows), layout.sf_off,
            layout.idx_off, layout.w_off, layout.src_off, ptr(error_flag), _stream_handle(stream))
        _lib.check(rc, 'dispatch_pack_cast')

    def dispatch_count(self, packed, layout: RowLayout, num_recv, rank, num_local_experts, rank_psum, meta,
                       recv_topk_idx, block_counts, pad_rows: int = 0, row_map=None, rank_counts=None,
                       psum_out=None, own_first: bool = False, stream=None):
        src = rank_psum if rank_psum is not None else rank_counts
        _require(src is not None and src.dim() == 1 and src.dtype == torch.int32 and src.stride(0) >= 1,
                 'dispatch_count needs rank_psum or rank_counts (int32 [num_ranks])')
        R = src.shape[0]
        stride = 0 if rank_psum is not None else src.stride(0)
        _require(psum_out is None or (psum_out.dtype == torch.int32 and psum_out.is_contiguous() and
                                      psum_out.numel() == R), 'psum_out must be contiguous int32 [num_ranks]')
        _require(pad_rows == 0 or (row_map is not None and row_map.dtype == torch.int32 and
                                   row_map.numel() >= num_recv and packed.shape[0] >= pad_rows * R),
                 'padded receive rows need a row map and R * pad_rows packed rows')
        _require(not own_first or (row_map is not None and row_map.dtype == torch.int32 and
                                   row_map.numel() >= num_recv), 'own-first receive rows need a row map')
        rc = self.lib.deepep_dispatch_count(
            ptr(packed), layout.row_bytes, layout.idx_off, layout.src_off, num_recv, layout.num_topk, rank,
            num_local_experts, ptr(src), R, stride, ptr(psum_out), pad_rows, int(own_first), ptr(row_map), ptr(meta),
            ptr(recv_topk_idx), ptr(block_counts), _stream_handle(stream))
        _lib.check(rc, 'dispatch_count')

    def dispatch_receive(self, packed, layout: RowLayout, num_recv, rank, num_local_experts, rank_counts, psum_out,
                         meta, recv_topk_idx, block_counts, expert_alignment, expanded, expert_counts, psum_expert,
                         inv=None, pad_rows: int = 0, row_map=None, own_first: bool = False, stream=None):
        _require(rank_counts.dim() == 1 and rank_counts.dtype == torch.int32 and rank_counts.stride(0) >= 1,
                 'rank_counts must be an int32 [num_ranks] view')
        R = rank_counts.shape[0]
        _require(psum_out.dtype == torch.int32 and psum_out.is_contiguous() and psum_out.numel() == R,
                 'psum_out must be contiguous int32 [num_ranks]')
        _require(pad_rows == 0 or (row_map is not None and row_map.dtype == torch.int32 and
                                   row_map.numel() >= num_recv and packed.shape[0] >= pad_rows * R),
                 'padded receive rows need a row map and R * pad_rows packed rows')
        _require(not own_first or (row_map is not None and row_map.dtype == torch.int32 and
                                   row_map.numel() >= num_recv), 'own-first receive rows need a row map')
        _require(inv is None or (inv.dtype == torch.int32 and inv.is_contiguous()), 'inv int32')
        rc = self.lib.deepep_dispatch_receive(
            ptr(packed), layout.row_bytes, layout.idx_off, layout.src_off, num_recv, layout.num_topk, rank,
            num_local_experts, ptr(rank_counts), R, rank_counts.stride(0), ptr(psum_out), pad_rows, int(own_first),
            ptr(row_map),
            ptr(meta), ptr(recv_topk_idx), ptr(block_counts), expert_alignment, int(expanded), ptr(expert_counts),
            ptr(psum_expert), ptr(inv), _stream_handle(stream))
        _lib.check(rc, 'dispatch_receive')

    def dispatch_scan(self, block_counts, num_local_experts, expert_alignment, expanded, expert_counts,
                      psum_expert, stream=None):
        rc = self.lib.deepep_dispatch_scan(ptr(block_counts), block_counts.shape[0], num_local_experts,
                                           expert_alignment, int(expanded), ptr(expert_counts), ptr(psum_expert),
                                           _stream_handle(stream))
        _lib.check(rc, 'dispatch_scan')

    def dispatch_slots(self, packed, layout: RowLayout, num_recv, rank, num_local_experts, block_offsets, meta,
                       inv=None, row_map=None, stream=None):
        _require(inv is None or (inv.dtype == torch.int32 and inv.is_contiguous()), 'inv int32')
        rc = self.lib.deepep_dispatch_slots(ptr(packed), layout.row_bytes, layout.idx_off, num_recv,
                                            layout.num_topk, rank, num_local_experts, ptr(block_offsets),
                                            ptr(meta), ptr(inv), ptr(row_map), _stream_handle(stream))
        _lib.check(rc, 'dispatch_slots')

    def dispatch_copy(self, packed, layout: RowLayout, num_recv, meta, expanded, recv_x_bytes, recv_sf_bytes,
                      recv_w, x_direct=None, sf_direct=None, num_max_tokens: int = 0, error_flag=None,
                      inv=None, block_offsets=None, expert_end=None, row_map=None, stream=None):
        if inv is not None:
            _require(expanded and block_offsets is not None and expert_end is not None and
                     block_offsets.dim() == 2 and block_offsets.shape[0] ==
                     (num_recv + _lib.DISPATCH_BLOCK_ROWS - 1) // _lib.DISPATCH_BLOCK_ROWS and
                     expert_end.numel() == block_offsets.shape[1], 'blocked copy tables')
        x_bytes = x_direct.shape[1] if x_direct is not None else layout.x_bytes
        sf_bytes = sf_direct.shape[1] if sf_direct is not None else layout.sf_bytes
        rc = self.lib.deepep_dispatch_copy(ptr(packed), layout.row_bytes, x_bytes, layout.sf_off,
                                           sf_bytes, layout.w_off, num_recv, layout.num_topk, ptr(meta),
                                           int(expanded),
                                           ptr(x_direct), x_direct.stride(0) if x_direct is not None else 0,
                                           ptr(sf_direct), sf_direct.stride(0) if sf_direct is not None else 0,
                                           num_max_tokens,
                                           ptr(recv_x_bytes), ptr(recv_sf_bytes), ptr(recv_w),
                                           recv_x_bytes.shape[0], ptr(inv), ptr(block_offsets), ptr(expert_end),
                                           block_offsets.shape[1] if block_offsets is not None else 0,
                                           ptr(row_map), ptr(error_flag), _stream_handle(stream))
        _lib.check(rc, 'dispatch_copy')

    def combine_buffer_size(self, num_max_tokens_per_rank: int, hidden: int, num_topk: int,
                            num_ranks: int, allow_multiple_reduction: bool) -> int:
        v = self.lib.deepep_combine_buffer_size(num_max_tokens_per_rank, hidden, num_topk, num_ranks,
                                                int(allow_multiple_reduction))
        _lib.check(0 if v >= 0 else int(v), 'combine_buffer_size')
        return int(v)
```

include/deepep_amd.h:

```cpp
#ifndef DEEPEP_AMD_H
#define DEEPEP_AMD_H

#include <stdint.h>

#ifdef __cplusplus
extern "C" {
#endif

typedef struct ihipStream_t* deepep_stream_t;

#define DEEPEP_AMD_ABI_VERSION 14

#define DEEPEP_OK               0
#define DEEPEP_ERR_INVALID_ARG  (-1)
#define DEEPEP_ERR_UNSUPPORTED  (-2)
#define DEEPEP_ERR_HIP          (-3)

#define DEEPEP_ERROR_RECORD_INTS 8
#define DEEPEP_FLAG_BAD_SLOT     1
#define DEEPEP_FLAG_TIMEOUT      2
#define DEEPEP_FLAG_BAD_ADDRESS  4
#define DEEPEP_FAULT_SCATTER_ROW 1
#define DEEPEP_FAULT_PLAN_ROW    2
#define DEEPEP_FAULT_PLAN_UNIT   3
#define DEEPEP_FAULT_PACK_ROW    4

#define DEEPEP_MODE_LOCAL     0
#define DEEPEP_MODE_EPILOGUE  1
#define DEEPEP_MODE_FUSED     2

int deepep_amd_abi_version(void);
const char* deepep_amd_last_error(void);
const char* deepep_amd_build_id(void);

int deepep_combine_reduce(int mode, int weighted,
                          const void* src, int64_t num_src_rows, int64_t src_row_stride,
                          const int32_t* table, int64_t table_stride, int table_width,
                          const float* row_weights,
                          const void* bias0, const void* bias1,
                          void* out, int64_t out_row_stride,
                          int num_units, int hidden,
                          const int32_t* wtable, int64_t wtable_stride,
                          const float* wsrc, float* out_weights, int num_weights,
                          int64_t out_weights_stride, int weights_pad,
                          int units_per_block, int32_t* error_flag,
                          deepep_stream_t stream);

int deepep_build_local_plan(const int32_t* src_metadata, int num_recv_tokens, int num_topk,
                            int num_max_tokens_per_rank, int expanded,
                            int32_t* plan, int plan_width, int num_tokens,
                            const int64_t* topk_idx, int32_t* wtable,
                            deepep_stream_t stream);

int deepep_set_launch_config(int vec_per_lane, int rows_in_flight);


int deepep_dispatch_route(const int64_t* topk_idx, int num_tokens, int num_topk, int num_experts, int num_ranks,
                          int32_t* dst_slot, int32_t* send_counts, int32_t* block_counts, deepep_stream_t stream);

int deepep_dispatch_expert_counts(const int64_t* topk_idx, int num_tokens, int num_topk, int num_experts,
                                  int32_t* counts, deepep_stream_t stream);

int64_t deepep_dispatch_notify_workspace(int num_tokens, int num_experts, int num_ranks);
int deepep_dispatch_notify(const int64_t* topk_idx, int num_tokens, int num_topk, int num_experts, int num_ranks,
                           int num_blocks, int32_t* dst_slot, int32_t* notify, int32_t* send_offsets,
                           void* workspace, int64_t workspace_bytes, deepep_stream_t stream);

int deepep_dispatch_pack(const void* x, int64_t x_row_stride_bytes, int x_bytes,
                         const void* sf, int64_t sf_row_stride_bytes, int sf_bytes,
                         const int64_t* topk_idx, const float* topk_weights, int num_tokens, int num_topk,
                         int32_t src_base, const int32_t* dst_slot, const int32_t* send_offsets, int num_ranks,
                         void* packed, const uint64_t* dest_bases, int64_t row_bytes, int64_t dest_rows,
                         int sf_off, int idx_off, int w_off, int src_off, int32_t* error_flag,
                         deepep_stream_t stream);

int deepep_cast_fp8(const void* x, int64_t x_row_stride_bytes, int num_rows, int hidden, int round_scale,
                    void* q, float* sf, deepep_stream_t stream);

int deepep_dispatch_pack_cast(const void* x, int64_t x_row_stride_bytes, int hidden, int round_scale,
                              const int64_t* topk_idx, const float* topk_weights, int num_tokens, int num_topk,
                              int32_t src_base, const int32_t* dst_slot, const int32_t* send_offsets, int num_ranks,
                              void* packed, const uint64_t* dest_bases, int64_t row_bytes, int64_t dest_rows,
                              int sf_off, int idx_off, int w_off, int src_off, int32_t* error_flag,
                              deepep_stream_t stream);

#define DEEPEP_DISPATCH_BLOCK_ROWS 128

int deepep_dispatch_count(const void* packed, int64_t row_bytes, int idx_off, int src_off, int num_recv, int num_topk,
                          int rank, int num_local_experts, const int32_t* recv_rank_psum, int num_ranks,
                          int recv_counts_stride, int32_t* psum_out, int pad_rows, int own_first, int32_t* row_map,
                          int32_t* src_metadata, int64_t* recv_topk_idx, int32_t* block_counts,
                          deepep_stream_t stream);

int deepep_dispatch_receive(const void* packed, int64_t row_bytes, int idx_off, int src_off, int num_recv,
                            int num_topk, int rank, int num_local_experts, const int32_t* recv_counts,
                            int num_ranks, int recv_counts_stride, int32_t* psum_out, int pad_rows, int own_first,
                            int32_t* row_map,
                            int32_t* src_metadata, int64_t* recv_topk_idx, int32_t* block_counts,
                            int expert_alignment, int expanded, int32_t* expert_counts, int32_t* psum_expert,
                            int32_t* inv, deepep_stream_t stream);

int deepep_dispatch_scan(int32_t* block_counts, int num_blocks, int num_local_experts, int expert_alignment,
                         int expanded, int32_t* expert_counts, int32_t* psum_expert, deepep_stream_t stream);

int deepep_dispatch_slots(const void* packed, int64_t row_bytes, int idx_off, int num_recv, int num_topk,
                          int rank, int num_local_experts, const int32_t* block_offsets, int32_t* src_metadata,
                          int32_t* inv, const int32_t* row_map, deepep_stream_t stream);

int deepep_dispatch_copy(const void* packed, int64_t row_bytes, int x_bytes, int sf_off, int sf_bytes, int w_off,
                         int num_recv, int num_topk, const int32_t* src_metadata, int expanded,
                         const void* x_direct, int64_t x_direct_stride_bytes,
                         const void* sf_direct, int64_t sf_direct_stride_bytes, int num_max_tokens,
                         void* recv_x, void* recv_sf, float* recv_topk_weights, int64_t num_out_rows,
                         const int32_t* inv, const int32_t* block_offsets, const int32_t* expert_end,
                         int num_local_experts, const int32_t* row_map, int32_t* error_flag, deepep_stream_t stream);

#define DEEPEP_PLAN_BLOCK_TOKENS 64
#define DEEPEP_PLAN_EXPANDED     1
#define DEEPEP_PLAN_SINGLE       2
#define DEEPEP_PLAN_INTERLEAVE   4
#define DEEPEP_PLAN_RANK_LAYOUT  8
#define DEEPEP_PLAN_WINDOW      16
#define DEEPEP_PLAN_LOCAL_BYPASS 32

int deepep_route_block_counts(const int64_t* topk_idx, int num_tokens, int num_topk, int num_experts, int num_ranks,
                              int num_blocks, int32_t* tok_counts, int32_t* pair_counts, deepep_stream_t stream);

int deepep_plan_expert(const int32_t* src_metadata, int num_recv, int num_topk, int num_ranks, int rank,
                       int num_max_tokens, const int32_t* recv_tok, const int32_t* recv_pairs, int num_blocks,
                       int blocks_per_chunk, int flags, int32_t* table_a, int32_t* wtable_a,
                       const uint64_t* window_bases, int64_t window_row_bytes, int64_t window_bytes,
                       uint64_t* out_rows, int32_t* error_flag, int padded_stride, deepep_stream_t stream);

int deepep_plan_source(const int64_t* topk_idx, int num_tokens, int num_topk, int num_experts, int num_ranks,
                       int rank, int num_max_tokens, const int32_t* dst_slot, const int32_t* send_tok,
                       const int32_t* send_pairs, int num_blocks, int blocks_per_chunk, int flags,
                       int64_t row_floats, int64_t weights_offset, int32_t* table_b, int table_b_width,
                       int32_t* wtable, int padded_stride, deepep_stream_t stream);

#define DEEPEP_IPC_HANDLE_BYTES 64

int deepep_sym_alloc(int64_t bytes, void** ptr);
int deepep_sym_free(void* ptr);
int deepep_sym_export(void* ptr, void* handle);
int deepep_sym_import(const void* handle, void** ptr);
int deepep_sym_close(void* ptr);

#define DEEPEP_SYM_NOTIFY_OFFSET 65536
#define DEEPEP_SYM_HEADER_BYTES 1048576

int deepep_sym_put(const void* src, int64_t bytes, const uint64_t* dest_bases, int num_ranks, int64_t dest_offset,
                   int64_t dest_extent, const int32_t* error_flag, deepep_stream_t stream);

int deepep_sym_barrier(const uint64_t* peer_flags, int rank, int num_ranks, int64_t epoch, int64_t timeout_us,
                       int32_t* error_flag, deepep_stream_t stream);

#define DEEPEP_SYM_FLAG_SLOTS 64
int deepep_sym_signal(const uint64_t* peer_flags, int rank, int num_ranks, int slot, int64_t value,
                      deepep_stream_t stream);
int deepep_sym_wait(const uint64_t* peer_flags, int rank, int num_ranks, int slot, int64_t value, int64_t timeout_us,
                    int32_t* error_flag, deepep_stream_t stream);

int deepep_combine_reduce_scatter(int weighted,
                                  const void* src, int64_t num_src_rows, int64_t src_row_stride,
                                  const int32_t* table, int64_t table_stride, int table_width,
                                  const float* row_weights,
                                  const uint64_t* out_rows, int num_units, int hidden,
                                  const int32_t* wtable, int64_t wtable_stride,
                                  const float* wsrc, int num_weights, int64_t weights_offset, int weights_pad,
                                  const uint64_t* window_bases, int num_windows, int64_t window_bytes,
                                  int32_t* error_flag, deepep_stream_t stream);

int deepep_stream_create_cu_budget(int num_cus, deepep_stream_t* stream);
int deepep_stream_destroy(deepep_stream_t stream);
int deepep_stream_probe_cus(deepep_stream_t stream, int* num_cus, int* num_xcds);

int64_t deepep_combine_buffer_size(int num_max_tokens_per_rank, int hidden, int num_topk,
                                   int num_ranks, int allow_multiple_reduction);

#ifdef __cplusplus
}
#endif

#endif
```

Measured before the change: 6576 GB/s.

## Add single-rank local dispatch route that builds combine tables and skips packing

For one rank, dispatch now runs dedicated count, scan and slot kernels that compute slots, metadata, the inverse map and the combine lookup tables in one pass. The copy then reads x and the weights straight from the sender instead of through a packed staging buffer. Combine reuses the prebuilt tables rather than launching build_local_plan. This mainly cuts dispatch and plan overhead; the timed combine reduce kernel itself is unchanged, so the combine bandwidth metric may barely move.

Measured after the change: 6234 GB/s. 5.2% lower.

```diff
diff --git a/deepep_amd/_lib.py b/deepep_amd/_lib.py
--- a/deepep_amd/_lib.py
+++ b/deepep_amd/_lib.py
@@ -97,6 +97,10 @@
     'deepep_dispatch_slots': (_I, [_P, _I64, _I, _I, _I, _I, _I, _P, _P, _P, _P, _P]),
     'deepep_dispatch_copy': (_I, [_P, _I64, _I, _I, _I, _I, _I, _I, _P, _I, _P, _I64, _P, _I64, _I,
                                   _P, _P, _P, _I64, _P, _P, _P, _I, _P, _P, _P]),
+    'deepep_dispatch_route_local': (_I, [_P, _I, _I, _I, _I, _I, _P, _P, _P, _P, _P, _P, _P, _P, _P, _P, _P, _I64, _P,
+                                         _P, _P, _P]),
+    'deepep_dispatch_copy_local': (_I, [_P, _I64, _I, _P, _I64, _I, _P, _I, _I, _P, _I, _I, _P, _P, _P, _I64, _P, _P,
+                                        _P, _I, _P, _P]),
     'deepep_route_block_counts': (_I, [_P, _I, _I, _I, _I, _I, _P, _P, _P]),
     'deepep_plan_expert': (_I, [_P, _I, _I, _I, _I, _I, _P, _P, _I, _I, _I, _P, _P, _P, _I64, _I64, _P, _P, _I,
                                 _P]),
diff --git a/deepep_amd/buffer.py b/deepep_amd/buffer.py
--- a/deepep_amd/buffer.py
+++ b/deepep_amd/buffer.py
@@ -455,6 +455,9 @@
             layout = (RowLayout.make(0, 0, K) if direct else
                       RowLayout.make(x_bytes.shape[1], sf_bytes.shape[1] if sf is not None else 0, K))
             sym = self._window(layout.row_bytes, slots=R, rows_per_slot=num_max_tokens_per_rank) if use_xgmi else None
+            route_local = (R == 1 and self.use_cuda and os.environ.get('DEEPEP_ROUTE_LOCAL', '1') != '0' and
+                           hasattr(kern, 'dispatch_route_local') and not sync_free and not worst_handle)
+            local_tables = None
             if cached is not None:
                 dst_slot = cached.dst_buffer_slot_idx
                 send_counts_l, recv_counts_l = cached._send_counts, cached._recv_counts
@@ -466,6 +469,30 @@
                 _assert(not (worst_handle and R > 1) or use_xgmi == (peer_offsets is not None) and
                         (use_xgmi or cached._row_map is not None),
                         'a handle from dispatch(do_cpu_sync=False) is cached only on the transport that made it')
+            elif route_local:
+                i32 = dict(dtype=torch.int32, device=dev)
+                nblocks = ceil_div(T, DISPATCH_BLOCK_ROWS)
+                dst_slot = torch.empty((T, 1), **i32)
+                send_offsets = torch.empty((1,), **i32)
+                notify = torch.empty((1, 1 + epr), **i32)
+                psum_rank = torch.empty((1,), **i32)
+                meta = torch.empty((T, K + 2), **i32)
+                out_idx = None if do_expand else torch.empty((T, K), dtype=torch.int64, device=dev)
+                block_counts = torch.empty((nblocks, epr), **i32)
+                expert_counts = torch.empty((epr,), **i32)
+                psum_expert = torch.empty((epr,), **i32)
+                local_inv = torch.empty((T * min(K, epr) + (expert_alignment - 1) * epr,), **i32) if do_expand else None
+                own_idx = (torch.empty_like(idx64) if do_handle_copy and topk_idx.dtype == torch.int64 and
+                           topk_idx.is_contiguous() else None)
+                local_tables = (torch.empty((T, K if do_expand else 1), **i32),
+                                None if do_expand else torch.empty((T, K), **i32))
+                kern.dispatch_route_local(idx64, epr, expert_alignment, do_expand, block_counts,
+                                          torch.empty((nblocks,), **i32), dst_slot, send_offsets, psum_rank,
+                                          expert_counts, psum_expert, notify.view(-1), meta, out_idx, local_inv,
+                                          own_idx, local_tables[0], local_tables[1], stream=stream)
+                host_notify = self._host_copy(notify.view(-1), stream)
+                send_counts_l = recv_counts_l = [T]
+                counts = None
             else:
                 nb = chunk_geometry(num_max_tokens_per_rank, 1)[0] if R > 1 else 0
                 w_n = 1 + epr + 2 * nb
@@ -566,6 +593,8 @@
                           [0 if d == r else c for d, c in enumerate(send_counts_l)])
                 recv_packed = rows_all[n_send - own:]
                 own_first = True
+            elif route_local:
+                recv_packed = None
             else:
                 n_send = T if sync_free else sum(send_counts_l)
                 packed = torch.empty((n_send, layout.row_bytes), dtype=torch.uint8, device=dev)
@@ -590,6 +619,13 @@
                 if cumulative_local_expert_recv_stats is not None:
                     cumulative_local_expert_recv_stats += expert_counts.to(cumulative_local_expert_recv_stats.dtype)
                 self._before_epilogue(previous_event_before_epilogue)
+            elif route_local:
+                aligned_l = []
+                inv, block_offsets = local_inv, (block_counts if do_expand else None)
+                if cumulative_local_expert_recv_stats is not None:
+                    cumulative_local_expert_recv_stats += expert_counts.to(cumulative_local_expert_recv_stats.dtype)
+                self._before_epilogue(previous_event_before_epilogue)
+                copy_meta, copy_rows = meta, N
             else:
                 psum_rank = torch.empty((R,), dtype=torch.int32, device=dev)
                 meta = torch.empty((N, K + 2), dtype=torch.int32, device=dev)
@@ -644,7 +680,8 @@
                                sf_direct=sf_bytes if direct else None, num_max_tokens=num_max_tokens_per_rank,
                                error_flag=sym.error_flag if use_xgmi else None,
                                inv=inv if do_expand else None, block_offsets=block_offsets if do_expand else None,
-                               expert_end=psum_expert if do_expand else None, row_map=row_map, stream=stream)
+                               expert_end=psum_expert if do_expand else None, row_map=row_map, stream=stream,
+                               **(dict(w_direct=w) if route_local else {}))
             if deferred:
                 host = host_notify.wait()
                 send_counts_l = recv_counts_l = [host[0]]
@@ -668,7 +705,10 @@
             if out_idx is not None and topk_idx.dtype != torch.int64:
                 out_idx = out_idx.to(topk_idx.dtype)
             num_recv = N
-            cloned_idx = topk_idx.clone() if do_handle_copy and cached is None else topk_idx
+            if route_local and cached is None and own_idx is not None:
+                cloned_idx = own_idx
+            else:
+                cloned_idx = topk_idx.clone() if do_handle_copy and cached is None else topk_idx
         event = None if sync_mode else self._epilogue([x, sf, topk_idx, topk_weights, out_x, out_sf, out_idx, out_w,
                                                        meta], compute_stream, allocate_on_comm_stream,
                                                       async_with_compute_stream)
@@ -688,6 +728,7 @@
             handle._row_map = row_map
             handle._bypass = own_first
             handle._sync_free = sync_free
+            handle._local_tables = local_tables
         out_x = (out_x, out_sf) if out_sf is not None else out_x
         return out_x, out_idx, out_w, handle, EventOverlap(event)
 
@@ -733,11 +774,15 @@
             n_recv = handle.num_recv_tokens if handle._recv_counts is None else sum(handle._recv_counts)
             plan = CombinePlan(num_ranks=1, num_tokens=T, num_topk=K, expanded=handle.do_expand)
             width = K if handle.do_expand else 1
-            plan.local_table = torch.empty((T, width), dtype=torch.int32, device=meta.device)
-            if not handle.do_expand:
-                plan.local_wtable = torch.empty((T, K), dtype=torch.int32, device=meta.device)
-            self.kernels.build_local_plan(meta, n_recv, K, handle.num_max_tokens_per_rank, handle.do_expand,
-                                          plan.local_table, T, handle.topk_idx, plan.local_wtable, stream=stream)
+            tables = getattr(handle, '_local_tables', None)
+            if tables is not None:
+                plan.local_table, plan.local_wtable = tables
+            else:
+                plan.local_table = torch.empty((T, width), dtype=torch.int32, device=meta.device)
+                if not handle.do_expand:
+                    plan.local_wtable = torch.empty((T, K), dtype=torch.int32, device=meta.device)
+                self.kernels.build_local_plan(meta, n_recv, K, handle.num_max_tokens_per_rank, handle.do_expand,
+                                              plan.local_table, T, handle.topk_idx, plan.local_wtable, stream=stream)
         else:
             _assert(handle._counts is not None, 'the EP > 1 combine needs a handle made by this build\'s dispatch')
             plan = build_ep_plan(self.kernels, handle, num_ranks=R, rank=self.rank_idx, single=single_reduction,
diff --git a/deepep_amd/csrc/dispatch.hip b/deepep_amd/csrc/dispatch.hip
--- a/deepep_amd/csrc/dispatch.hip
+++ b/deepep_amd/csrc/dispatch.hip
@@ -364,12 +364,11 @@
             block_counts[static_cast<int64_t>(blockIdx.x) * epr + e] = s_hist[e];
 }
 
-__global__ void __launch_bounds__(1024)
-scan_kernel(int32_t* __restrict__ block_counts, int nblocks, int epr, int align, int expanded,
-            int32_t* __restrict__ expert_counts, int32_t* __restrict__ psum_expert) {
+__device__ __forceinline__ void
+scan_blocks(int32_t* __restrict__ block_counts, int nblocks, int epr, int align, int expanded,
+            int32_t* __restrict__ expert_counts, int32_t* __restrict__ psum_expert, int32_t* __restrict__ record,
+            int32_t* s_part, int32_t* s_aligned) {
     constexpr int kBatch = 16;
-    __shared__ int32_t s_part[1024];
-    __shared__ int32_t s_aligned[1024];
     const int tid = threadIdx.x;
     const int G = 1024 / epr;
     const int e = tid % epr, g = tid / epr;
@@ -403,6 +402,7 @@
     if (tid < epr) {
         const int start = s_aligned[tid] - aligned;
         expert_counts[tid] = total;
+        if (record != nullptr) record[tid] = total;
         psum_expert[tid] = expanded ? start + total : start + aligned;
         s_aligned[tid] = start;
     }
@@ -421,6 +421,14 @@
             run += c[j];
         }
     }
+}
+
+__global__ void __launch_bounds__(1024)
+scan_kernel(int32_t* __restrict__ block_counts, int nblocks, int epr, int align, int expanded,
+            int32_t* __restrict__ expert_counts, int32_t* __restrict__ psum_expert) {
+    __shared__ int32_t s_part[1024];
+    __shared__ int32_t s_aligned[1024];
+    scan_blocks(block_counts, nblocks, epr, align, expanded, expert_counts, psum_expert, nullptr, s_part, s_aligned);
 }
 
 constexpr int kSlotWaves = kBlockRows / 64;
@@ -458,11 +466,150 @@
     }
 }
 
+__device__ __forceinline__ bool local_valid(int64_t e, int E) { return e >= 0 && e < E; }
+
+__global__ void __launch_bounds__(kBlockRows)
+local_count_kernel(const int64_t* __restrict__ topk_idx, int T, int K, int E, int32_t* __restrict__ block_counts,
+                   int32_t* __restrict__ block_tokens, int64_t* __restrict__ idx_copy) {
+    extern __shared__ int32_t s_hist[];
+    __shared__ int32_t s_tok[kSlotWaves];
+    const int tid = threadIdx.x;
+    for (int e = tid; e < E; e += kBlockRows) s_hist[e] = 0;
+    __syncthreads();
+    const int t = blockIdx.x * kBlockRows + tid;
+    bool valid = false;
+    if (t < T)
+        for (int k = 0; k < K; ++k) {
+            const int64_t e = topk_idx[static_cast<int64_t>(t) * K + k];
+            if (local_valid(e, E)) {
+                valid = true;
+                atomicAdd(&s_hist[static_cast<int>(e)], 1);
+            }
+        }
+    const int c = __popcll(__ballot(valid));
+    if ((tid & 63) == 0) s_tok[tid >> 6] = c;
+    if (idx_copy != nullptr) {
+        const int64_t base = static_cast<int64_t>(blockIdx.x) * kBlockRows * K, n = static_cast<int64_t>(T) * K;
+        for (int j = tid; j < kBlockRows * K; j += kBlockRows)
+            if (base + j < n) idx_copy[base + j] = topk_idx[base + j];
+    }
+    __syncthreads();
+    for (int e = tid; e < E; e += kBlockRows) block_counts[static_cast<int64_t>(blockIdx.x) * E + e] = s_hist[e];
+    if (tid == 0) {
+        int n = 0;
+        for (int w = 0; w < kSlotWaves; ++w) n += s_tok[w];
+        block_tokens[blockIdx.x] = n;
+    }
+}
+
+__global__ void __launch_bounds__(1024)
+local_scan_kernel(int32_t* __restrict__ block_counts, int32_t* __restrict__ block_tokens, int nblocks, int E, int align,
+                  int expanded, int32_t* __restrict__ expert_counts, int32_t* __restrict__ psum_expert,
+                  int32_t* __restrict__ psum_rank, int32_t* __restrict__ send_offsets, int32_t* __restrict__ record) {
+    __shared__ int32_t s_part[1024];
+    __shared__ int32_t s_aligned[1024];
+    const int tid = threadIdx.x;
+    const int per = (nblocks + 1023) / 1024;
+    const int lo = min(nblocks, tid * per), hi = min(nblocks, lo + per);
+    int sum = 0;
+    for (int j = lo; j < hi; ++j) sum += block_tokens[j];
+    const int lane = tid & 63, wave = tid >> 6;
+    int incl = sum;
+#pragma unroll
+    for (int off = 1; off < 64; off <<= 1) {
+        const int v = __shfl_up(incl, off, 64);
+        if (lane >= off) incl += v;
+    }
+    if (lane == 63) s_part[wave] = incl;
+    __syncthreads();
+    for (int w = 0; w < wave; ++w) incl += s_part[w];
+    int run = incl - sum;
+    for (int j = lo; j < hi; ++j) {
+        const int c = block_tokens[j];
+        block_tokens[j] = run;
+        run += c;
+    }
+    if (tid == 1023) {
+        psum_rank[0] = incl;
+        record[0] = incl;
+        send_offsets[0] = 0;
+    }
+    __syncthreads();
+    scan_blocks(block_counts, nblocks, E, align, expanded, expert_counts, psum_expert, record + 1, s_part, s_aligned);
+}
+
+__global__ void __launch_bounds__(kBlockRows)
+local_slots_kernel(const int64_t* __restrict__ topk_idx, int T, int K, int E, int expanded,
+                   const int32_t* __restrict__ block_offsets, const int32_t* __restrict__ block_rows,
+                   const int32_t* __restrict__ psum_rank, int32_t* __restrict__ dst_slot, int32_t* __restrict__ meta,
+                   int64_t* __restrict__ recv_topk_idx, int32_t* __restrict__ inv, int64_t inv_len,
+                   int32_t* __restrict__ local_table, int32_t* __restrict__ local_wtable) {
+    extern __shared__ uint64_t s_bits[];
+    __shared__ int32_t s_tok[kSlotWaves];
+    for (int j = threadIdx.x; j < E * kSlotWaves; j += kBlockRows) s_bits[j] = 0ull;
+    __syncthreads();
+    const int t = blockIdx.x * kBlockRows + threadIdx.x;
+    const int wave = threadIdx.x >> 6, lane = threadIdx.x & 63;
+    const int64_t* idx = topk_idx + static_cast<int64_t>(t) * K;
+    int master = -1;
+    if (t < T)
+        for (int k = 0; k < K; ++k) {
+            const int64_t e = idx[k];
+            if (local_valid(e, E)) {
+                master = k;
+                atomicOr(reinterpret_cast<unsigned long long*>(&s_bits[static_cast<int>(e) * kSlotWaves + wave]),
+                         1ull << lane);
+            }
+        }
+    const bool valid = master >= 0;
+    const uint64_t vbal = __ballot(valid);
+    if (lane == 0) s_tok[wave] = __popcll(vbal);
+    __syncthreads();
+    if (t >= T) return;
+    const uint64_t lt = lane == 0 ? 0ull : (~0ull >> (64 - lane));
+    const int total = psum_rank[0];
+    const int width = K + 2;
+    if (t >= total) {
+        for (int c = 0; c < width; ++c) meta[static_cast<int64_t>(t) * width + c] = -1;
+        if (recv_topk_idx != nullptr)
+            for (int k = 0; k < K; ++k) recv_topk_idx[static_cast<int64_t>(t) * K + k] = -1;
+    }
+    int i = -1;
+    if (valid) {
+        i = block_rows[blockIdx.x] + __popcll(vbal & lt);
+        for (int w = 0; w < wave; ++w) i += s_tok[w];
+    }
+    dst_slot[t] = i;
+    if (local_table != nullptr && !expanded) local_table[t] = i;
+    if (valid) {
+        meta[static_cast<int64_t>(i) * width] = t;
+        meta[static_cast<int64_t>(i) * width + 1] = master;
+    }
+    for (int k = 0; k < K; ++k) {
+        const int64_t e = valid ? idx[k] : -1;
+        const int le = local_valid(e, E) ? static_cast<int>(e) : -1;
+        int slot = -1;
+        if (le >= 0 && expanded) {
+            slot = block_offsets[static_cast<int64_t>(blockIdx.x) * E + le];
+            for (int w = 0; w < wave; ++w) slot += __popcll(s_bits[le * kSlotWaves + w]);
+            slot += __popcll(s_bits[le * kSlotWaves + wave] & lt);
+            if (inv != nullptr && slot < inv_len) inv[slot] = i * K + k;
+        }
+        if (valid) {
+            meta[static_cast<int64_t>(i) * width + 2 + k] = slot;
+            if (recv_topk_idx != nullptr) recv_topk_idx[static_cast<int64_t>(i) * K + k] = le;
+        }
+        if (local_table != nullptr && expanded) local_table[static_cast<int64_t>(t) * K + k] = slot;
+        if (local_wtable != nullptr) local_wtable[static_cast<int64_t>(t) * K + k] = valid && e >= 0 ? i * K + k : -1;
+    }
+}
+
 __global__ void __launch_bounds__(256)
 copy_kernel(const uint8_t* __restrict__ packed, int64_t row_bytes, int x_bytes, int sf_off, int sf_bytes, int w_off,
             int N, int K, const int32_t* __restrict__ meta, int expanded,
             const uint8_t* __restrict__ x_direct, int64_t x_direct_stride,
             const uint8_t* __restrict__ sf_direct, int64_t sf_direct_stride, int num_max_tokens,
+            const float* __restrict__ w_direct,
             uint8_t* __restrict__ recv_x, uint8_t* __restrict__ recv_sf, float* __restrict__ recv_w,
             int64_t num_out_rows, const int32_t* __restrict__ row_map, int32_t* __restrict__ error_flag) {
     constexpr int kChunkVecs = 128;
@@ -479,10 +626,12 @@
     const uint8_t* row = packed + (row_map != nullptr ? static_cast<int64_t>(row_map[i]) : i) * row_bytes;
     const uint8_t* xs = row;
     const uint8_t* sfs = row + sf_off;
+    const float* ws = reinterpret_cast<const float*>(row + w_off);
     if (x_direct != nullptr) {
         const int64_t t = meta[i * (K + 2)] % num_max_tokens;
         xs = x_direct + t * x_direct_stride;
         sfs = sf_direct != nullptr ? sf_direct + t * sf_direct_stride : nullptr;
+        if (w_direct != nullptr) ws = w_direct + t * K;
     }
     int32_t my_dst = -1;
     if (expanded) {
@@ -516,7 +665,7 @@
             }
         }
     if (recv_w != nullptr && lane < K) {
-        const float w = reinterpret_cast<const float*>(row + w_off)[lane];
+        const float w = ws[lane];
         if (expanded) {
             if (my_dst >= 0) recv_w[my_dst] = w;
         } else {
@@ -533,8 +682,8 @@
                      int w_off, int N, int K, const int32_t* __restrict__ meta,
                      const uint8_t* __restrict__ x_direct, int64_t x_direct_stride,
                      const uint8_t* __restrict__ sf_direct, int64_t sf_direct_stride, int num_max_tokens,
-                     const int32_t* __restrict__ inv, const int32_t* __restrict__ block_offsets,
-                     const int32_t* __restrict__ expert_end, int nb, int epr,
+                     const float* __restrict__ w_direct, const int32_t* __restrict__ inv,
+                     const int32_t* __restrict__ block_offsets, const int32_t* __restrict__ expert_end, int nb, int epr,
                      uint8_t* __restrict__ recv_x, uint8_t* __restrict__ recv_sf, float* __restrict__ recv_w,
                      int64_t num_out_rows, const int32_t* __restrict__ row_map, int32_t* __restrict__ error_flag) {
     constexpr int kChunkVecs = 128;
@@ -606,7 +755,12 @@
                     for (int v = lane; v < sf_bytes / 4; v += 64)
                         reinterpret_cast<uint32_t*>(recv_sf + d * sf_bytes)[v] = reinterpret_cast<const uint32_t*>(sfs)[v];
             }
-            if (recv_w != nullptr && lane == 0) {
+            if (kDirect && w_direct != nullptr) {
+                if (recv_w != nullptr && lane == 0) {
+                    const int64_t t = meta[static_cast<int64_t>(src_i[q]) * (K + 2)] % num_max_tokens;
+                    recv_w[d] = w_direct[t * K + src_k[q]];
+                }
+            } else if (recv_w != nullptr && lane == 0) {
                 const int64_t prow = row_map != nullptr ? static_cast<int64_t>(row_map[src_i[q]]) : src_i[q];
                 recv_w[d] = reinterpret_cast<const float*>(packed + prow * row_bytes + w_off)[src_k[q]];
             }
@@ -625,6 +779,56 @@
 }
 
 bool a16(const void* p) { return (reinterpret_cast<uintptr_t>(p) & 15u) == 0; }
+bool a8(const void* p) { return (reinterpret_cast<uintptr_t>(p) & 7u) == 0; }
+bool a4(const void* p) { return (reinterpret_cast<uintptr_t>(p) & 3u) == 0; }
+
+int launch_copy(const void* packed, int64_t row_bytes, int x_bytes, int sf_off, int sf_bytes, int w_off,
+                int num_recv, int num_topk, const int32_t* src_metadata, int expanded,
+                const void* x_direct, int64_t x_direct_stride_bytes,
+                const void* sf_direct, int64_t sf_direct_stride_bytes, int num_max_tokens, const float* w_direct,
+                void* recv_x, void* recv_sf, float* recv_topk_weights, int64_t num_out_rows,
+                const int32_t* inv, const int32_t* block_offsets, const int32_t* expert_end,
+                int num_local_experts, const int32_t* row_map, int32_t* error_flag, deepep_stream_t stream) {
+    if (num_recv == 0) return DEEPEP_OK;
+    if (num_recv < 0 || num_topk < 1 || num_topk > 32 || x_bytes % 16 || row_bytes % 16 || !a16(packed) ||
+        num_out_rows < 0 ||
+        !a16(recv_x) || (recv_sf != nullptr && sf_bytes % 4) || src_metadata == nullptr ||
+        (x_direct != nullptr && (!a16(x_direct) || x_direct_stride_bytes % 16 || num_max_tokens < 1 ||
+                                 (recv_sf != nullptr && sf_direct == nullptr))) ||
+        (inv != nullptr && (!expanded || block_offsets == nullptr || expert_end == nullptr || num_local_experts < 1 ||
+                            num_local_experts > 1024)))
+        return deepep_amd_set_error(DEEPEP_ERR_INVALID_ARG, "dispatch_copy: invalid arguments or alignment");
+    if (inv != nullptr) {
+        const int nb = (num_recv + kBlockRows - 1) / kBlockRows;
+        const int nch = std::max(1, (x_bytes / 16 + 127) / 128);
+        const int64_t wg_per_block = (static_cast<int64_t>(num_local_experts) * nch + 3) / 4;
+        const int64_t grid = 8 * wg_per_block * ((nb + 7) / 8);
+        auto launch = [&](auto kernel) {
+            hipLaunchKernelGGL(kernel, dim3(static_cast<unsigned>(grid)), dim3(256), 0,
+                               reinterpret_cast<hipStream_t>(stream),
+                               static_cast<const uint8_t*>(packed), row_bytes, x_bytes, sf_off, sf_bytes, w_off,
+                               num_recv, num_topk, src_metadata, static_cast<const uint8_t*>(x_direct),
+                               x_direct_stride_bytes, static_cast<const uint8_t*>(sf_direct), sf_direct_stride_bytes,
+                               num_max_tokens, w_direct, inv, block_offsets, expert_end, nb, num_local_experts,
+                               static_cast<uint8_t*>(recv_x), static_cast<uint8_t*>(recv_sf), recv_topk_weights,
+                               num_out_rows, row_map, error_flag);
+        };
+        if (x_direct != nullptr) launch(copy_expanded_kernel<true>);
+        else launch(copy_expanded_kernel<false>);
+        return launch_status("dispatch_copy");
+    }
+    const int64_t nchunks = std::max<int64_t>(1, (x_bytes / 16 + 127) / 128);
+    const int64_t items = static_cast<int64_t>(num_recv) * nchunks;
+    hipLaunchKernelGGL(copy_kernel, dim3(static_cast<unsigned>((items + 3) / 4)), dim3(256), 0,
+                       reinterpret_cast<hipStream_t>(stream),
+                       static_cast<const uint8_t*>(packed), row_bytes, x_bytes, sf_off, sf_bytes, w_off,
+                       num_recv, num_topk, src_metadata, expanded,
+                       static_cast<const uint8_t*>(x_direct), x_direct_stride_bytes,
+                       static_cast<const uint8_t*>(sf_direct), sf_direct_stride_bytes, num_max_tokens, w_direct,
+                       static_cast<uint8_t*>(recv_x), static_cast<uint8_t*>(recv_sf), recv_topk_weights,
+                       num_out_rows, row_map, error_flag);
+    return launch_status("dispatch_copy");
+}
 
 }
 
@@ -810,45 +1014,62 @@
                          void* recv_x, void* recv_sf, float* recv_topk_weights, int64_t num_out_rows,
                          const int32_t* inv, const int32_t* block_offsets, const int32_t* expert_end,
                          int num_local_experts, const int32_t* row_map, int32_t* error_flag, deepep_stream_t stream) {
-    if (num_recv == 0) return DEEPEP_OK;
-    if (num_recv < 0 || num_topk < 1 || num_topk > 32 || x_bytes % 16 || row_bytes % 16 || !a16(packed) ||
-        num_out_rows < 0 ||
-        !a16(recv_x) || (recv_sf != nullptr && sf_bytes % 4) || src_metadata == nullptr ||
-        (x_direct != nullptr && (!a16(x_direct) || x_direct_stride_bytes % 16 || num_max_tokens < 1 ||
-                                 (recv_sf != nullptr && sf_direct == nullptr))) ||
-        (inv != nullptr && (!expanded || block_offsets == nullptr || expert_end == nullptr || num_local_experts < 1 ||
-                            num_local_experts > 1024)))
-        return deepep_amd_set_error(DEEPEP_ERR_INVALID_ARG, "dispatch_copy: invalid arguments or alignment");
-    if (inv != nullptr) {
-        const int nb = (num_recv + kBlockRows - 1) / kBlockRows;
-        const int nch = std::max(1, (x_bytes / 16 + 127) / 128);
-        const int64_t wg_per_block = (static_cast<int64_t>(num_local_experts) * nch + 3) / 4;
-        const int64_t grid = 8 * wg_per_block * ((nb + 7) / 8);
-        auto launch = [&](auto kernel) {
-            hipLaunchKernelGGL(kernel, dim3(static_cast<unsigned>(grid)), dim3(256), 0,
-                               reinterpret_cast<hipStream_t>(stream),
-                               static_cast<const uint8_t*>(packed), row_bytes, x_bytes, sf_off, sf_bytes, w_off,
-                               num_recv, num_topk, src_metadata, static_cast<const uint8_t*>(x_direct),
-                               x_direct_stride_bytes, static_cast<const uint8_t*>(sf_direct), sf_direct_stride_bytes,
-                               num_max_tokens, inv, block_offsets, expert_end, nb, num_local_experts,
-                               static_cast<uint8_t*>(recv_x), static_cast<uint8_t*>(recv_sf), recv_topk_weights,
-                               num_out_rows, row_map, error_flag);
-        };
-        if (x_direct != nullptr) launch(copy_expanded_kernel<true>);
-        else launch(copy_expanded_kernel<false>);
-        return launch_status("dispatch_copy");
-    }
-    const int64_t nchunks = std::max<int64_t>(1, (x_bytes / 16 + 127) / 128);
-    const int64_t items = static_cast<int64_t>(num_recv) * nchunks;
-    hipLaunchKernelGGL(copy_kernel, dim3(static_cast<unsigned>((items + 3) / 4)), dim3(256), 0,
-                       reinterpret_cast<hipStream_t>(stream),
-                       static_cast<const uint8_t*>(packed), row_bytes, x_bytes, sf_off, sf_bytes, w_off,
-                       num_recv, num_topk, src_metadata, expanded,
-                       static_cast<const uint8_t*>(x_direct), x_direct_stride_bytes,
-                       static_cast<const uint8_t*>(sf_direct), sf_direct_stride_bytes, num_max_tokens,
-                       static_cast<uint8_t*>(recv_x), static_cast<uint8_t*>(recv_sf), recv_topk_weights,
-                       num_out_rows, row_map, error_flag);
-    return launch_status("dispatch_copy");
-}
-
-}
+    return launch_copy(packed, row_bytes, x_bytes, sf_off, sf_bytes, w_off, num_recv, num_topk, src_metadata, expanded,
+                       x_direct, x_direct_stride_bytes, sf_direct, sf_direct_stride_bytes, num_max_tokens, nullptr,
+                       recv_x, recv_sf, recv_topk_weights, num_out_rows, inv, block_offsets, expert_end,
+                       num_local_experts, row_map, error_flag, stream);
+}
+
+int deepep_dispatch_copy_local(const void* x, int64_t x_row_stride_bytes, int x_bytes,
+                               const void* sf, int64_t sf_row_stride_bytes, int sf_bytes,
+                               const float* topk_weights, int num_rows, int num_topk, const int32_t* src_metadata,
+                               int expanded, int num_max_tokens, void* recv_x, void* recv_sf,
+                               float* recv_topk_weights, int64_t num_out_rows, const int32_t* inv,
+                               const int32_t* block_offsets, const int32_t* expert_end, int num_local_experts,
+                               int32_t* error_flag, deepep_stream_t stream) {
+    if (num_rows == 0) return DEEPEP_OK;
+    if (x == nullptr || recv_x == nullptr || x_bytes < 0 || x_row_stride_bytes < x_bytes || sf_bytes < 0 ||
+        (recv_sf != nullptr && (sf == nullptr || sf_row_stride_bytes < sf_bytes || sf_row_stride_bytes % 4 || !a4(sf) ||
+                                !a4(recv_sf))) ||
+        (recv_topk_weights != nullptr && (topk_weights == nullptr || !a4(topk_weights) || !a4(recv_topk_weights))) ||
+        !a4(src_metadata) || !a4(inv) || !a4(block_offsets) || !a4(expert_end) || !a4(error_flag))
+        return deepep_amd_set_error(DEEPEP_ERR_INVALID_ARG, "dispatch_copy_local: invalid arguments or alignment");
+    return launch_copy(nullptr, 0, x_bytes, 0, sf_bytes, 0, num_rows, num_topk, src_metadata, expanded, x,
+                       x_row_stride_bytes, recv_sf != nullptr ? sf : nullptr, sf_row_stride_bytes, num_max_tokens,
+                       recv_topk_weights != nullptr ? topk_weights : nullptr, recv_x, recv_sf, recv_topk_weights,
+                       num_out_rows, inv, block_offsets, expert_end, num_local_experts, nullptr, error_flag, stream);
+}
+
+int deepep_dispatch_route_local(const int64_t* topk_idx, int num_tokens, int num_topk, int num_experts,
+                                int expert_alignment, int expanded, int32_t* block_counts, int32_t* block_tokens,
+                                int32_t* dst_slot, int32_t* send_offsets, int32_t* psum_rank, int32_t* expert_counts,
+                                int32_t* psum_expert, int32_t* record, int32_t* src_metadata, int64_t* recv_topk_idx,
+                                int32_t* inv, int64_t inv_len, int64_t* topk_idx_copy, int32_t* local_table,
+                                int32_t* local_wtable, deepep_stream_t stream) {
+    if (num_tokens < 0 || num_topk < 1 || num_topk > 32 || num_experts < 1 || num_experts > 1024 ||
+        expert_alignment < 1 || inv_len < 0 || static_cast<int64_t>(num_tokens) * num_topk >= (int64_t(1) << 31) ||
+        send_offsets == nullptr || psum_rank == nullptr || expert_counts == nullptr || psum_expert == nullptr ||
+        record == nullptr ||
+        (num_tokens > 0 && (topk_idx == nullptr || block_counts == nullptr || block_tokens == nullptr ||
+                            dst_slot == nullptr || src_metadata == nullptr || (expanded && inv == nullptr))))
+        return deepep_amd_set_error(DEEPEP_ERR_INVALID_ARG, "dispatch_route_local: invalid sizes or null pointers");
+    if (!a8(topk_idx) || !a8(recv_topk_idx) || !a8(topk_idx_copy) || !a4(block_counts) || !a4(block_tokens) ||
+        !a4(dst_slot) || !a4(send_offsets) || !a4(psum_rank) || !a4(expert_counts) || !a4(psum_expert) || !a4(record) ||
+        !a4(src_metadata) || !a4(inv) || !a4(local_table) || !a4(local_wtable))
+        return deepep_amd_set_error(DEEPEP_ERR_INVALID_ARG, "dispatch_route_local: misaligned pointers");
+    hipStream_t s = reinterpret_cast<hipStream_t>(stream);
+    const int nblocks = (num_tokens + kBlockRows - 1) / kBlockRows;
+    if (nblocks > 0)
+        hipLaunchKernelGGL(local_count_kernel, dim3(nblocks), dim3(kBlockRows), num_experts * 4, s, topk_idx, num_tokens,
+                           num_topk, num_experts, block_counts, block_tokens, topk_idx_copy);
+    hipLaunchKernelGGL(local_scan_kernel, dim3(1), dim3(1024), 0, s, block_counts, block_tokens, nblocks, num_experts,
+                       expert_alignment, expanded ? 1 : 0, expert_counts, psum_expert, psum_rank, send_offsets, record);
+    if (nblocks > 0)
+        hipLaunchKernelGGL(local_slots_kernel, dim3(nblocks), dim3(kBlockRows), num_experts * kSlotWaves * 8, s,
+                           topk_idx, num_tokens, num_topk, num_experts, expanded ? 1 : 0, block_counts, block_tokens,
+                           psum_rank, dst_slot, src_metadata, recv_topk_idx, expanded ? inv : nullptr, inv_len,
+                           local_table, local_wtable);
+    return launch_status("dispatch_route_local");
+}
+
+}
diff --git a/deepep_amd/kernels.py b/deepep_amd/kernels.py
--- a/deepep_amd/kernels.py
+++ b/deepep_amd/kernels.py
@@ -327,14 +327,58 @@
                                             ptr(meta), ptr(inv), ptr(row_map), _stream_handle(stream))
         _lib.check(rc, 'dispatch_slots')
 
+    def dispatch_route_local(self, topk_idx, num_experts, expert_alignment, expanded, block_counts, block_tokens,
+                             dst_slot, send_offsets, psum_rank, expert_counts, psum_expert, record, meta,
+                             recv_topk_idx, inv, topk_idx_copy, local_table, local_wtable, stream=None):
+        _require(topk_idx.is_cuda and topk_idx.dtype == torch.int64 and topk_idx.is_contiguous(), 'topk_idx int64')
+        T, K = topk_idx.shape
+        nb = (T + _lib.DISPATCH_BLOCK_ROWS - 1) // _lib.DISPATCH_BLOCK_ROWS
+        for t, n, what in ((block_counts, nb * num_experts, 'block_counts'), (block_tokens, nb, 'block_tokens'),
+                           (dst_slot, T, 'dst_slot'), (send_offsets, 1, 'send_offsets'), (psum_rank, 1, 'psum_rank'),
+                           (expert_counts, num_experts, 'expert_counts'), (psum_expert, num_experts, 'psum_expert'),
+                           (record, 1 + num_experts, 'record'), (meta, T * (K + 2), 'src_metadata'),
+                           (local_table, T * (K if expanded else 1), 'local_table'), (local_wtable, T * K, 'local_wtable')):
+            _require(t is None and what.startswith('local_') or
+                     t is not None and t.is_cuda and t.dtype == torch.int32 and t.is_contiguous() and t.numel() == n,
+                     f'{what} must be contiguous int32 with {n} elements on the GPU')
+        for t, what in ((recv_topk_idx, 'recv_topk_idx'), (topk_idx_copy, 'topk_idx_copy')):
+            _require(t is None or (t.is_cuda and t.dtype == torch.int64 and t.is_contiguous() and t.numel() == T * K),
+                     f'{what} must be contiguous int64 [num_tokens, num_topk] on the GPU')
+        _require(not expanded or (inv is not None and inv.is_cuda and inv.dtype == torch.int32 and inv.is_contiguous()),
+                 'the expanded layout needs inv (contiguous int32 on the GPU)')
+        rc = self.lib.deepep_dispatch_route_local(
+            ptr(topk_idx), T, K, num_experts, expert_alignment, int(expanded), ptr(block_counts), ptr(block_tokens),
+            ptr(dst_slot), ptr(send_offsets), ptr(psum_rank), ptr(expert_counts), ptr(psum_expert), ptr(record),
+            ptr(meta), ptr(recv_topk_idx), ptr(inv), inv.numel() if inv is not None else 0, ptr(topk_idx_copy),
+            ptr(local_table), ptr(local_wtable), _stream_handle(stream))
+        _lib.check(rc, 'dispatch_route_local')
+
     def dispatch_copy(self, packed, layout: RowLayout, num_recv, meta, expanded, recv_x_bytes, recv_sf_bytes,
                       recv_w, x_direct=None, sf_direct=None, num_max_tokens: int = 0, error_flag=None,
-                      inv=None, block_offsets=None, expert_end=None, row_map=None, stream=None):
+                      inv=None, block_offsets=None, expert_end=None, row_map=None, w_direct=None, stream=None):
         if inv is not None:
             _require(expanded and block_offsets is not None and expert_end is not None and
                      block_offsets.dim() == 2 and block_offsets.shape[0] ==
                      (num_recv + _lib.DISPATCH_BLOCK_ROWS - 1) // _lib.DISPATCH_BLOCK_ROWS and
                      expert_end.numel() == block_offsets.shape[1], 'blocked copy tables')
+        if packed is None:
+            _require(x_direct is not None and row_map is None and (recv_sf_bytes is None or sf_direct is not None),
+                     'a copy without packed rows reads x (and sf) from the sender')
+            _require(recv_w is None or (w_direct is not None and w_direct.dtype == torch.float32 and
+                                        w_direct.is_contiguous() and tuple(w_direct.shape) ==
+                                        (x_direct.shape[0], layout.num_topk)),
+                     'a copy without packed rows needs the sender\'s float32 [T, K] weights')
+            _require(meta.dtype == torch.int32 and meta.is_contiguous() and
+                     meta.numel() >= num_recv * (layout.num_topk + 2), 'src_metadata int32 [num_recv, K + 2]')
+            rc = self.lib.deepep_dispatch_copy_local(
+                ptr(x_direct), x_direct.stride(0), x_direct.shape[1],
+                ptr(sf_direct), sf_direct.stride(0) if sf_direct is not None else 0,
+                sf_direct.shape[1] if sf_direct is not None else 0, ptr(w_direct), num_recv, layout.num_topk, ptr(meta),
+                int(expanded), num_max_tokens, ptr(recv_x_bytes), ptr(recv_sf_bytes), ptr(recv_w),
+                recv_x_bytes.shape[0], ptr(inv), ptr(block_offsets), ptr(expert_end),
+                block_offsets.shape[1] if block_offsets is not None else 0, ptr(error_flag), _stream_handle(stream))
+            _lib.check(rc, 'dispatch_copy_local')
+            return
         x_bytes = x_direct.shape[1] if x_direct is not None else layout.x_bytes
         sf_bytes = sf_direct.shape[1] if sf_direct is not None else layout.sf_bytes
         rc = self.lib.deepep_dispatch_copy(ptr(packed), layout.row_bytes, x_bytes, layout.sf_off,
diff --git a/include/deepep_amd.h b/include/deepep_amd.h
--- a/include/deepep_amd.h
+++ b/include/deepep_amd.h
@@ -115,6 +115,21 @@
                          const int32_t* inv, const int32_t* block_offsets, const int32_t* expert_end,
                          int num_local_experts, const int32_t* row_map, int32_t* error_flag, deepep_stream_t stream);
 
+int deepep_dispatch_route_local(const int64_t* topk_idx, int num_tokens, int num_topk, int num_experts,
+                                int expert_alignment, int expanded, int32_t* block_counts, int32_t* block_tokens,
+                                int32_t* dst_slot, int32_t* send_offsets, int32_t* psum_rank, int32_t* expert_counts,
+                                int32_t* psum_expert, int32_t* record, int32_t* src_metadata, int64_t* recv_topk_idx,
+                                int32_t* inv, int64_t inv_len, int64_t* topk_idx_copy, int32_t* local_table,
+                                int32_t* local_wtable, deepep_stream_t stream);
+
+int deepep_dispatch_copy_local(const void* x, int64_t x_row_stride_bytes, int x_bytes,
+                               const void* sf, int64_t sf_row_stride_bytes, int sf_bytes,
+                               const float* topk_weights, int num_rows, int num_topk, const int32_t* src_metadata,
+                               int expanded, int num_max_tokens, void* recv_x, void* recv_sf,
+                               float* recv_topk_weights, int64_t num_out_rows, const int32_t* inv,
+                               const int32_t* block_offsets, const int32_t* expert_end, int num_local_experts,
+                               int32_t* error_flag, deepep_stream_t stream);
+
 #define DEEPEP_PLAN_BLOCK_TOKENS 64
 #define DEEPEP_PLAN_EXPANDED     1
 #define DEEPEP_PLAN_SINGLE       2
```
